# Shigangli/Ok-Topk

Hardware: NVIDIA H100
Metric: train_samples_per_sec_vgg16_oktopk_density0.001 (higher is better)
Workload: dtype fp32

## Files before the change

oktopk_b200/csrc/bindings.cpp:

```cpp
#include <pybind11/pybind11.h>
#include <pybind11/stl.h>
#include <cuda.h>
#include <cuda_runtime.h>

#include <unistd.h>

#include <algorithm>
#include <cstring>
#include <stdexcept>
#include <string>
#include <tuple>
#include <vector>

#include "oktopk.cuh"

namespace py = pybind11;
using namespace okt;

static void ck(cudaError_t e, const char* what) {
    if (e != cudaSuccess) throw std::runtime_error(std::string(what) + ": " + cudaGetErrorString(e));
}
template <class T> static T* P_(uint64_t p) { return reinterpret_cast<T*>(p); }
static cudaStream_t S_(uint64_t s) { return reinterpret_cast<cudaStream_t>(s); }

static py::tuple symm_alloc(size_t nbytes) {
    void* p = nullptr;
    ck(cudaMalloc(&p, nbytes), "cudaMalloc(symm)");
    ck(cudaMemset(p, 0, nbytes), "cudaMemset(symm)");
    cudaIpcMemHandle_t h;
    ck(cudaIpcGetMemHandle(&h, p), "cudaIpcGetMemHandle");
    return py::make_tuple((uint64_t)p, py::bytes(reinterpret_cast<const char*>(&h), sizeof(h)));
}
static uint64_t symm_open(const std::string& handle) {
    if (handle.size() != sizeof(cudaIpcMemHandle_t)) throw std::runtime_error("bad IPC handle size");
    cudaIpcMemHandle_t h;
    std::memcpy(&h, handle.data(), sizeof(h));
    void* p = nullptr;
    ck(cudaIpcOpenMemHandle(&p, h, cudaIpcMemLazyEnablePeerAccess), "cudaIpcOpenMemHandle");
    return (uint64_t)p;
}
static void symm_close(uint64_t p) { ck(cudaIpcCloseMemHandle(P_<void>(p)), "cudaIpcCloseMemHandle"); }
static void symm_free(uint64_t p) { ck(cudaFree(P_<void>(p)), "cudaFree(symm)"); }
static uint64_t dev_alloc_zero(size_t nbytes) {
    void* p = nullptr;
    ck(cudaMalloc(&p, nbytes), "cudaMalloc");
    ck(cudaMemset(p, 0, nbytes), "cudaMemset");
    return (uint64_t)p;
}
static void dev_free(uint64_t p) {
    if (p) ck(cudaFree(P_<void>(p)), "cudaFree");
}
static void memset_async(uint64_t p, int value, size_t nbytes, uint64_t stream) {
    ck(cudaMemsetAsync(P_<void>(p), value, nbytes, S_(stream)), "cudaMemsetAsync");
}
static int can_access_peer(int dev, int peer) {
    int ok = 0;
    ck(cudaDeviceCanAccessPeer(&ok, dev, peer), "cudaDeviceCanAccessPeer");
    return ok;
}


namespace drv {
template <class F> static F sym(const char* name) {
    void* fn = nullptr;
    cudaDriverEntryPointQueryResult q;
    cudaError_t e = cudaGetDriverEntryPoint(name, &fn, cudaEnableDefault, &q);
    if (e != cudaSuccess || fn == nullptr || q != cudaDriverEntryPointSuccess)
        throw std::runtime_error(std::string("driver entry point not available: ") + name);
    return reinterpret_cast<F>(fn);
}
static void ckd(CUresult r, const char* what) {
    if (r != CUDA_SUCCESS) throw std::runtime_error(std::string(what) + ": CUresult " + std::to_string((int)r));
}
}

static CUmemAllocationProp vmm_prop(int dev) {
    CUmemAllocationProp prop;
    std::memset(&prop, 0, sizeof(prop));
    prop.type = CU_MEM_ALLOCATION_TYPE_PINNED;
    prop.location.type = CU_MEM_LOCATION_TYPE_DEVICE;
    prop.location.id = dev;
    prop.requestedHandleTypes = CU_MEM_HANDLE_TYPE_POSIX_FILE_DESCRIPTOR;
    return prop;
}

static py::dict vmm_probe(int dev, int ndev) {
    py::dict d;
    d["vmm"] = 0; d["posix_fd"] = 0; d["multicast"] = 0; d["granularity"] = 0; d["mc_granularity"] = 0;
    try {
        auto getattr_ = drv::sym<CUresult (*)(int*, CUdevice_attribute, CUdevice)>("cuDeviceGetAttribute");
        int v = 0;
        if (getattr_(&v, CU_DEVICE_ATTRIBUTE_VIRTUAL_MEMORY_MANAGEMENT_SUPPORTED, dev) == CUDA_SUCCESS) d["vmm"] = v;
        if (getattr_(&v, CU_DEVICE_ATTRIBUTE_HANDLE_TYPE_POSIX_FILE_DESCRIPTOR_SUPPORTED, dev) == CUDA_SUCCESS) d["posix_fd"] = v;
        if (getattr_(&v, CU_DEVICE_ATTRIBUTE_MULTICAST_SUPPORTED, dev) == CUDA_SUCCESS) d["multicast"] = v;
        auto gran = drv::sym<CUresult (*)(size_t*, const CUmemAllocationProp*, CUmemAllocationGranularity_flags)>("cuMemGetAllocationGranularity");
        CUmemAllocationProp prop = vmm_prop(dev);
        size_t g = 0;
        if (gran(&g, &prop, CU_MEM_ALLOC_GRANULARITY_RECOMMENDED) == CUDA_SUCCESS) d["granularity"] = g;
        if (d["multicast"].cast<int>() && ndev > 1) {
            auto mgran = drv::sym<CUresult (*)(size_t*, const CUmulticastObjectProp*, CUmulticastGranularity_flags)>("cuMulticastGetGranularity");
            CUmulticastObjectProp mp;
            std::memset(&mp, 0, sizeof(mp));
            mp.numDevices = ndev; mp.size = 1 << 21; mp.handleTypes = CU_MEM_HANDLE_TYPE_POSIX_FILE_DESCRIPTOR;
            size_t mg = 0;
            if (mgran(&mg, &mp, CU_MULTICAST_GRANULARITY_RECOMMENDED) == CUDA_SUCCESS) d["mc_granularity"] = mg;
        }
    } catch (const std::exception& e) {
        d["error"] = std::string(e.what());
    }
    return d;
}

static py::tuple vmm_create(size_t nbytes, int dev) {
    auto create = drv::sym<CUresult (*)(CUmemGenericAllocationHandle*, size_t, const CUmemAllocationProp*, unsigned long long)>("cuMemCreate");
    auto exp = drv::sym<CUresult (*)(void*, CUmemGenericAllocationHandle, CUmemAllocationHandleType, unsigned long long)>("cuMemExportToShareableHandle");
    CUmemAllocationProp prop = vmm_prop(dev);
    CUmemGenericAllocationHandle h = 0;
    drv::ckd(create(&h, nbytes, &prop, 0), "cuMemCreate");
    int fd = -1;
    drv::ckd(exp(&fd, h, CU_MEM_HANDLE_TYPE_POSIX_FILE_DESCRIPTOR, 0), "cuMemExportToShareableHandle");
    return py::make_tuple((uint64_t)h, fd);
}
static uint64_t vmm_import(int fd) {
    auto imp = drv::sym<CUresult (*)(CUmemGenericAllocationHandle*, void*, CUmemAllocationHandleType)>("cuMemImportFromShareableHandle");
    CUmemGenericAllocationHandle h = 0;
    drv::ckd(imp(&h, reinterpret_cast<void*>(static_cast<uintptr_t>(fd)), CU_MEM_HANDLE_TYPE_POSIX_FILE_DESCRIPTOR), "cuMemImportFromShareableHandle");
    return (uint64_t)h;
}
static uint64_t vmm_map(uint64_t handle, size_t nbytes, int dev, size_t align) {
    auto reserve = drv::sym<CUresult (*)(CUdeviceptr*, size_t, size_t, CUdeviceptr, unsigned long long)>("cuMemAddressReserve");
    auto map = drv::sym<CUresult (*)(CUdeviceptr, size_t, size_t, CUmemGenericAllocationHandle, unsigned long long)>("cuMemMap");
    auto access = drv::sym<CUresult (*)(CUdeviceptr, size_t, const CUmemAccessDesc*, size_t)>("cuMemSetAccess");
    CUdeviceptr va = 0;
    drv::ckd(reserve(&va, nbytes, align, 0, 0), "cuMemAddressReserve");
    drv::ckd(map(va, nbytes, 0, (CUmemGenericAllocationHandle)handle, 0), "cuMemMap");
    CUmemAccessDesc ad;
    std::memset(&ad, 0, sizeof(ad));
    ad.location.type = CU_MEM_LOCATION_TYPE_DEVICE;
    ad.location.id = dev;
    ad.flags = CU_MEM_ACCESS_FLAGS_PROT_READWRITE;
    drv::ckd(access(va, nbytes, &ad, 1), "cuMemSetAccess");
    return (uint64_t)va;
}
static void vmm_unmap(uint64_t va, size_t nbytes) {
    auto unmap = drv::sym<CUresult (*)(CUdeviceptr, size_t)>("cuMemUnmap");
    auto afree = drv::sym<CUresult (*)(CUdeviceptr, size_t)>("cuMemAddressFree");
    unmap((CUdeviceptr)va, nbytes);
    afree((CUdeviceptr)va, nbytes);
}
static void vmm_release(uint64_t handle) {
    auto rel = drv::sym<CUresult (*)(CUmemGenericAllocationHandle)>("cuMemRelease");
    rel((CUmemGenericAllocationHandle)handle);
}
static py::tuple mc_create(size_t nbytes, int ndev) {
    auto create = drv::sym<CUresult (*)(CUmemGenericAllocationHandle*, const CUmulticastObjectProp*)>("cuMulticastCreate");
    auto exp = drv::sym<CUresult (*)(void*, CUmemGenericAllocationHandle, CUmemAllocationHandleType, unsigned long long)>("cuMemExportToShareableHandle");
    CUmulticastObjectProp mp;
    std::memset(&mp, 0, sizeof(mp));
    mp.numDevices = ndev; mp.size = nbytes; mp.handleTypes = CU_MEM_HANDLE_TYPE_POSIX_FILE_DESCRIPTOR;
    CUmemGenericAllocationHandle h = 0;
    drv::ckd(create(&h, &mp), "cuMulticastCreate");
    int fd = -1;
    drv::ckd(exp(&fd, h, CU_MEM_HANDLE_TYPE_POSIX_FILE_DESCRIPTOR, 0), "cuMemExportToShareableHandle(mc)");
    return py::make_tuple((uint64_t)h, fd);
}
static void mc_add_device(uint64_t mc, int dev) {
    auto add = drv::sym<CUresult (*)(CUmemGenericAllocationHandle, CUdevice)>("cuMulticastAddDevice");
    drv::ckd(add((CUmemGenericAllocationHandle)mc, dev), "cuMulticastAddDevice");
}
static void mc_bind(uint64_t mc, uint64_t mem, size_t nbytes) {
    auto bind = drv::sym<CUresult (*)(CUmemGenericAllocationHandle, size_t, CUmemGenericAllocationHandle, size_t, size_t, unsigned long long)>("cuMulticastBindMem");
    drv::ckd(bind((CUmemGenericAllocationHandle)mc, 0, (CUmemGenericAllocationHandle)mem, 0, nbytes, 0), "cuMulticastBindMem");
}

static size_t state_bytes() { return sizeof(OktState); }

static py::dict layout_info(int P, int n, int cap, int gcap) {
    SymmLayout L = make_layout(P, n, cap, gcap);
    py::dict d;
    d["total"] = L.total; d["rs_mbox"] = L.rs_mbox; d["rs_thr"] = L.rs_thr; d["ag_mbox"] = L.ag_mbox;
    d["cut_mbox"] = L.cut_mbox; d["cut_data"] = L.cut_data; d["send_idx"] = L.send_idx; d["send_val"] = L.send_val;
    d["gat_idx"] = L.gat_idx; d["gat_val"] = L.gat_val; d["cap"] = L.cap; d["gcap"] = L.gcap; d["scap"] = L.scap;
    d["done_mbox"] = L.done_mbox; d["tree_mbox"] = L.tree_mbox;
    d["chunk"] = kChunk; d["maxp"] = OKT_MAXP; d["threads"] = kThreads;
    return d;
}

static py::dict read_state(uint64_t st, int P, uint64_t stream) {
    static thread_local std::vector<char> host(offsetof(OktState, hist));
    ck(cudaMemcpyAsync(host.data(), P_<void>(st), host.size(), cudaMemcpyDeviceToHost, S_(stream)), "read_state");
    ck(cudaStreamSynchronize(S_(stream)), "read_state sync");
    const OktState* s = reinterpret_cast<const OktState*>(host.data());
    py::dict d;
    d["local_thr"] = s->local_thr; d["local_thr_used"] = s->local_thr_used; d["global_thr"] = s->global_thr;
    d["epoch"] = s->epoch;
    std::vector<int> e(s->edges, s->edges + P + 1);
    d["edges"] = e;
    d["local_count"] = s->stat_local_count; d["global_count"] = s->stat_global_count;
    d["recv_total"] = s->stat_recv_total; d["gather_total"] = s->stat_gather_total;
    d["overflow_send"] = s->stat_overflow_send; d["overflow_gather"] = s->stat_overflow_gather;
    d["redo"] = s->stat_redo; d["dense_fallback"] = s->stat_dense_fallback; d["pack_thr"] = s->pack_thr;
    d["cum_overflow_send"] = s->cum_overflow_send; d["cum_overflow_gather"] = s->cum_overflow_gather;
    d["cum_redo"] = s->cum_redo;
    d["fault"] = s->fault;
    auto us = [&](int a, int b) { return s->t_phase[b] >= s->t_phase[a] ? (double)(s->t_phase[b] - s->t_phase[a]) * 1e-3 : 0.0; };
    py::dict ph;
    ph["local"] = us(5, 0); ph["pack"] = us(0, 1); ph["wait_rs"] = us(1, 6); ph["reduce"] = us(6, 2); ph["gselect"] = us(2, 3);
    ph["wait_ag"] = us(3, 7); ph["final"] = us(7, 4); ph["total"] = us(5, 4);
    d["phase_us"] = ph;
    return d;
}

static py::list read_trace(uint64_t st, uint64_t stream) {
    std::vector<TraceRec> host(kTraceLen);
    ck(cudaMemcpyAsync(host.data(), reinterpret_cast<char*>(P_<OktState>(st)) + offsetof(OktState, trace),
                       sizeof(TraceRec) * kTraceLen, cudaMemcpyDeviceToHost, S_(stream)), "read_trace");
    ck(cudaStreamSynchronize(S_(stream)), "read_trace sync");
    py::list out;
    for (const TraceRec& t : host) {
        if (t.epoch == 0) continue;
        py::dict d;
        d["epoch"] = t.epoch; d["local_count"] = t.local_count; d["global_count"] = t.global_count;
        d["recv_total"] = t.recv_total; d["gather_total"] = t.gather_total; d["overflow_send"] = t.overflow_send;
        d["overflow_gather"] = t.overflow_gather; d["redo"] = t.redo; d["local_thr"] = t.local_thr;
        d["global_thr"] = t.global_thr; d["us_local"] = t.us_local; d["us_pack"] = t.us_pack;
        d["us_wait_rs"] = t.us_wait_rs; d["us_reduce"] = t.us_reduce; d["us_gselect"] = t.us_gselect;
        d["us_wait_ag"] = t.us_wait_ag; d["us_final"] = t.us_final; d["t_begin"] = t.t_begin;
        out.append(d);
    }
    return out;
}

static py::tuple host_flag_alloc() {
    int* h = nullptr;
    ck(cudaHostAlloc(reinterpret_cast<void**>(&h), sizeof(int) * 16, cudaHostAllocMapped), "cudaHostAlloc(flag)");
    for (int i = 0; i < 16; ++i) h[i] = 0;
    void* d = nullptr;
    ck(cudaHostGetDevicePointer(&d, h, 0), "cudaHostGetDevicePointer");
    return py::make_tuple((uint64_t)h, (uint64_t)d);
}
static void host_flag_free(uint64_t h) { if (h) cudaFreeHost(P_<void>(h)); }
static int host_flag_read(uint64_t h) { return h ? *reinterpret_cast<volatile int*>(h) : 0; }
static void host_flag_clear(uint64_t h) { if (h) *reinterpret_cast<volatile int*>(h) = 0; }

static void write_state(uint64_t st, float local_thr, float global_thr, const std::vector<int>& edges, uint64_t stream) {
    std::vector<char> host(offsetof(OktState, hist));
    ck(cudaMemcpyAsync(host.data(), P_<void>(st), host.size(), cudaMemcpyDeviceToHost, S_(stream)), "write_state rd");
    ck(cudaStreamSynchronize(S_(stream)), "write_state sync");
    OktState* s = reinterpret_cast<OktState*>(host.data());
    s->local_thr = local_thr;
    s->global_thr = global_thr;
    if (!edges.empty()) {
        if (edges.size() > OKT_MAXP + 1) throw std::runtime_error("too many region edges");
        for (size_t i = 0; i < edges.size(); ++i) s->edges[i] = edges[i];
    }
    ck(cudaMemcpyAsync(P_<void>(st), host.data(), host.size(), cudaMemcpyHostToDevice, S_(stream)), "write_state wr");
    ck(cudaStreamSynchronize(S_(stream)), "write_state sync2");
}

static void fill_peers(char** dst, const std::vector<uint64_t>& peers) {
    if (peers.size() > OKT_MAXP) throw std::runtime_error("world larger than OKT_MAXP");
    for (int i = 0; i < OKT_MAXP; ++i) dst[i] = nullptr;
    for (size_t i = 0; i < peers.size(); ++i) dst[i] = P_<char>(peers[i]);
}

static void oktopk_run(uint64_t g, uint64_t res, uint64_t st, const std::vector<uint64_t>& peers, int n, int rank,
                       int k, int cap, int gcap, py::dict o, int grid, uint64_t stream) {
    OktParams p;
    std::memset(&p, 0, sizeof(p));
    p.g = P_<float>(g); p.res = P_<float>(res); p.st = P_<OktState>(st);
    if (!o.contains("cand") || !o.contains("ccap")) throw std::runtime_error("oktopk_run: candidate scratch missing");
    p.cand = P_<int>(o["cand"].cast<uint64_t>()); p.ccap = o["ccap"].cast<int>();
    p.cand_mode = o.contains("cand_mode") ? o["cand_mode"].cast<int>() : 1;
    fill_peers(p.peers, peers);
    p.P = (int)peers.size(); p.rank = rank; p.n = n; p.k = k;
    p.L = make_layout(p.P, n, cap, gcap);
    auto geti = [&](const char* key, int dflt) { return o.contains(key) ? o[key].cast<int>() : dflt; };
    auto getf = [&](const char* key, double dflt) { return o.contains(key) ? o[key].cast<double>() : dflt; };
    for (int i = 0; i < OKT_MAXP; ++i) p.peer_g[i] = nullptr;
    if (o.contains("peer_g")) {
        auto pg = o["peer_g"].cast<std::vector<uint64_t>>();
        for (size_t i = 0; i < pg.size() && i < OKT_MAXP; ++i) p.peer_g[i] = P_<float>(pg[i]);
    }
    p.max_redo = geti("max_redo", 12);
    p.redo_factor = (float)getf("redo_factor", 1.5);
    p.dense_nnz_limit = geti("dense_nnz_limit", 0);
    p.host_fault = o.contains("host_fault") ? P_<int>(o["host_fault"].cast<uint64_t>()) : nullptr;
    p.trace = geti("trace", 0);
    p.exact_local = geti("exact_local", 0);
    p.repartition = geti("repartition", 0);
    p.uniform_regions = geti("uniform_regions", 0);
    p.residual_mode = geti("residual_mode", RES_OKTOPK);
    p.global_mode = geti("global_mode", GLB_THRESHOLD);
    p.deterministic = geti("deterministic", 0);
    p.pull_tma = geti("pull_tma", 1);
    p.phase_begin = geti("phase_begin", 0);
    p.phase_end = geti("phase_end", PH_END);
    p.guard_loops = geti("guard_loops", 0);
    if (p.guard_loops > kGuardFineMax) p.guard_loops = kGuardFineMax;
    p.cap_limit = geti("cap_limit", 0);
    p.cap_rungs = geti("cap_rungs", 40);
    p.cap_factor = (float)getf("cap_factor", 1.19);
    p.guard_limit = geti("guard_limit", 0);
    p.guard_factor = (float)getf("guard_factor", 1.03);
    p.l_low_cnt = getf("l_low_cnt", 0.0); p.l_high_cnt = getf("l_high_cnt", 1e30);
    p.l_factor = (float)getf("l_factor", 1.012);
    p.g_low_cnt = getf("g_low_cnt", 0.0); p.g_high_cnt = getf("g_high_cnt", 1e30);
    p.g_inc = (float)getf("g_inc", 1.008); p.g_dec = (float)getf("g_dec", 1.008);
    p.prefilter = (float)getf("prefilter", 0.8);
    p.timeout_ns = (unsigned long long)(getf("timeout_s", 0.0) * 1e9);
    if (o.contains("srcs")) {
        auto t = o["srcs"].cast<std::tuple<std::vector<uint64_t>, std::vector<long long>, std::vector<long long>>>();
        const auto& ptr = std::get<0>(t);
        const auto& off = std::get<1>(t);
        const auto& len = std::get<2>(t);
        if (off.size() != ptr.size() || len.size() != ptr.size()) throw std::runtime_error("oktopk_run: srcs table size mismatch");
        if (ptr.size() > (size_t)kSrcSegMax) throw std::runtime_error("oktopk_run: more gradient sources than kSrcSegMax");
        long long end = 0;
        for (size_t i = 0; i < ptr.size(); ++i) {
            if (off[i] < end || (off[i] & 3) || len[i] <= 0 || off[i] + len[i] > n || (ptr[i] & 15))
                throw std::runtime_error("oktopk_run: gradient sources must be 16-byte aligned, in bucket order, "
                                         "non-overlapping, at offsets that are multiples of 4 elements");
            p.src[i] = P_<const float>(ptr[i]);
            p.src_off[i] = (int)off[i];
            p.src_len[i] = (int)len[i];
            end = off[i] + len[i];
        }
        p.nsrc = (int)ptr.size();
        p.zero_g = 0;
    } else {
        if (g & 15) throw std::runtime_error("oktopk_run: the bucket must be 16-byte aligned");
        p.src[0] = P_<const float>(g);
        p.src_off[0] = 0;
        p.src_len[0] = n;
        p.nsrc = 1;
        p.zero_g = 1;
    }
    if (geti("split_phases", 0)) {
        for (int ph = p.phase_begin; ph < p.phase_end; ++ph) {
            OktParams q = p;
            q.phase_begin = ph; q.phase_end = ph + 1;
            ck(launch_oktopk(q, grid, S_(stream)), "oktopk phase launch");
        }
    } else {
        ck(launch_oktopk(p, grid, S_(stream)), "oktopk fused launch");
    }
}

static void gather_run(uint64_t g, uint64_t res, uint64_t st, const std::vector<uint64_t>& peers, int n, int rank,
                       int k, int cap, int gcap, py::dict o, int grid, uint64_t stream) {
    GatherParams p;
    std::memset(&p, 0, sizeof(p));
    p.g = P_<float>(g); p.res = P_<float>(res); p.st = P_<OktState>(st);
    fill_peers(p.peers, peers);
    p.P = (int)peers.size(); p.rank = rank; p.n = n; p.k = k;
    p.L = make_layout(p.P, n, cap, gcap);
    p.reselect = o.contains("reselect") ? o["reselect"].cast<int>() : 0;
    p.clip_max_norm = o.contains("clip_max_norm") ? (float)o["clip_max_norm"].cast<double>() : 0.f;
    p.bitmap = o.contains("bitmap") ? P_<unsigned>(o["bitmap"].cast<uint64_t>()) : nullptr;
    p.cand = o.contains("cand") ? P_<int>(o["cand"].cast<uint64_t>()) : nullptr;
    p.ccap = o.contains("ccap") ? o["ccap"].cast<int>() : 0;
    p.host_fault = o.contains("host_fault") ? P_<int>(o["host_fault"].cast<uint64_t>()) : nullptr;
    if (p.reselect && (p.bitmap == nullptr || p.cand == nullptr || p.ccap <= 0))
        throw std::runtime_error("gather_run: TopkA2 needs the bitmap and candidate scratch");
    p.select_mode = o["select_mode"].cast<int>();
    p.exact_now = o.contains("exact_now") ? o["exact_now"].cast<int>() : 0;
    p.gauss_mode = o.contains("gauss_mode") ? o["gauss_mode"].cast<int>() : 0;
    p.gauss_loops = o.contains("gauss_loops") ? o["gauss_loops"].cast<int>() : 20;
    p.gauss_factor = o.contains("gauss_factor") ? (float)o["gauss_factor"].cast<double>() : 1.02f;
    p.density = (float)o["density"].cast<double>();
    p.pull_tma = o.contains("pull_tma") ? o["pull_tma"].cast<int>() : 1;
    p.timeout_ns = o.contains("timeout_s") ? (unsigned long long)(o["timeout_s"].cast<double>() * 1e9) : 0ULL;
    ck(launch_gather_scheme(p, grid, S_(stream)), "gather scheme launch");
}

static void gtopk_run(uint64_t g, uint64_t res, uint64_t st, const std::vector<uint64_t>& peers, int n, int rank,
                      int k, int cap, int gcap, py::dict o, int grid, uint64_t stream) {
    TreeParams p;
    std::memset(&p, 0, sizeof(p));
    p.g = P_<float>(g); p.res = P_<float>(res); p.st = P_<OktState>(st);
    fill_peers(p.peers, peers);
    p.P = (int)peers.size(); p.rank = rank; p.n = n; p.k = k;
    if (p.P & (p.P - 1)) throw std::runtime_error("gTopk needs a power-of-two world size (VGG/allreducer.py:113)");
    p.L = make_layout(p.P, n, cap, gcap);
    p.pull_tma = o.contains("pull_tma") ? o["pull_tma"].cast<int>() : 1;
    p.timeout_ns = o.contains("timeout_s") ? (unsigned long long)(o["timeout_s"].cast<double>() * 1e9) : 0ULL;
    p.clip_max_norm = o.contains("clip_max_norm") ? (float)o["clip_max_norm"].cast<double>() : 0.f;
    p.bitmap = P_<unsigned>(o["bitmap"].cast<uint64_t>());
    p.cand = P_<int>(o["cand"].cast<uint64_t>());
    p.ccap = o["ccap"].cast<int>();
    p.sel_idx = P_<int>(o["sel_idx"].cast<uint64_t>());
    p.sel_val = P_<float>(o["sel_val"].cast<uint64_t>());
    p.selcap = o["selcap"].cast<int>();
    p.host_fault = o.contains("host_fault") ? P_<int>(o["host_fault"].cast<uint64_t>()) : nullptr;
    ck(launch_gtopk(p, grid, S_(stream)), "gtopk launch");
}

static void land_grads(const std::vector<uint64_t>& srcs, const std::vector<long long>& offs, const std::vector<int>& numels,
                       uint64_t bucket, uint64_t stream) {
    const size_t T = srcs.size();
    if (offs.size() != T || numels.size() != T) throw std::runtime_error("land_grads: table size mismatch");
    constexpr int per = 8192;
    for (size_t b = 0; b < T; b += kLandMax) {
        LandParams lp;
        std::memset(&lp, 0, sizeof(lp));
        const int cnt = (int)std::min<size_t>(kLandMax, T - b);
        int blk = 0;
        for (int i = 0; i < cnt; ++i) {
            lp.src[i] = P_<const float>(srcs[b + i]);
            lp.dst_off[i] = offs[b + i];
            lp.numel[i] = numels[b + i];
            lp.blk_begin[i] = blk;
            blk += std::max(1, (numels[b + i] + per - 1) / per);
        }
        lp.blk_begin[cnt] = blk;
        lp.count = cnt;
        ck(launch_land(lp, P_<float>(bucket), S_(stream)), "land_grads");
    }
}

static void dense_run(const std::vector<uint64_t>& bufs, const std::vector<uint64_t>& flags, uint64_t epoch, int n,
                      int rank, int grid, uint64_t stream, uint64_t st, double timeout_s, uint64_t mc,
                      uint64_t host_fault) {
    DenseParams p;
    std::memset(&p, 0, sizeof(p));
    if (bufs.size() > OKT_MAXP || bufs.size() != flags.size()) throw std::runtime_error("bad peer tables");
    for (size_t i = 0; i < bufs.size(); ++i) { p.bufs[i] = P_<float>(bufs[i]); p.flags[i] = P_<uint64_t>(flags[i]); }
    p.epoch = P_<unsigned long long>(epoch);
    p.n = n; p.P = (int)bufs.size(); p.rank = rank; p.scale = 1.0f / (float)p.P;
    p.fault = st ? &P_<OktState>(st)->fault : nullptr;
    p.timeout_ns = (unsigned long long)(timeout_s * 1e9);
    p.mc = P_<float>(mc);
    p.host_fault = P_<int>(host_fault);
    ck(launch_dense_allreduce(p, grid, S_(stream)), "dense allreduce launch");
}

static void kth_abs(uint64_t x, int n, int k, uint64_t st, uint64_t out, int grid, uint64_t stream) {
    ck(launch_kth_abs(P_<float>(x), n, k, P_<OktState>(st), P_<float>(out), grid, S_(stream)), "kth_abs launch");
}

static void fused_sgd(uint64_t p, uint64_t g, uint64_t mom, int n, double lr, double momentum, double dampening,
                      double wd, int nesterov, int first, int zero_grad, double grad_scale, uint64_t stream,
                      uint64_t lr_ptr, uint64_t fault_ptr) {
    ck(launch_fused_sgd(P_<float>(p), P_<float>(g), P_<float>(mom), n, (float)lr, (float)momentum, (float)dampening,
                        (float)wd, nesterov, first, zero_grad, (float)grad_scale, P_<float>(lr_ptr), P_<int>(fault_ptr),
                        S_(stream)),
       "fused_sgd");
}
static void fused_bert_adam(uint64_t p, uint64_t g, uint64_t m, uint64_t v, int n, double lr, double b1, double b2,
                            double eps, double wd, int zero_grad, uint64_t stream, uint64_t lr_ptr, uint64_t fault_ptr) {
    ck(launch_fused_bert_adam(P_<float>(p), P_<float>(g), P_<float>(m), P_<float>(v), n, (float)lr, (float)b1,
                              (float)b2, (float)eps, (float)wd, zero_grad, P_<float>(lr_ptr), P_<int>(fault_ptr),
                              S_(stream)),
       "fused_bert_adam");
}
static void bn_forward(uint64_t x, uint64_t y, uint64_t arg, uint64_t partial, uint64_t gamma, uint64_t beta, uint64_t cbias,
                       uint64_t save_mean, uint64_t save_invstd, uint64_t rmean, uint64_t rvar, uint64_t nbt, double momentum,
                       double eps, int relu, int M, int C, int W, int slot, int max_ctas, uint64_t stream) {
    if (C % 4 != 0) throw std::runtime_error("bn_forward: channel count must be a multiple of 4");
    if (slot < 0) throw std::runtime_error("bn_forward: negative slot");
    ck(launch_bn_forward(P_<const float>(x), P_<float>(y), P_<unsigned char>(arg), P_<float>(partial), P_<const float>(gamma),
                         P_<const float>(beta), P_<const float>(cbias), P_<float>(save_mean), P_<float>(save_invstd),
                         P_<float>(rmean), P_<float>(rvar), P_<long long>(nbt), (float)momentum, (float)eps, relu, M, C, W, slot,
                         max_ctas, S_(stream)), "bn_forward");
}
static void bn_backward(uint64_t x, uint64_t dy, uint64_t arg, uint64_t dx, uint64_t partial, uint64_t gamma, uint64_t beta,
                        uint64_t save_mean, uint64_t save_invstd, uint64_t dgamma, uint64_t dbeta, int relu, int M, int C, int W,
                        int slot, int max_ctas, uint64_t stream) {
    if (slot < 0) throw std::runtime_error("bn_backward: negative slot");
    ck(launch_bn_backward(P_<const float>(x), P_<const float>(dy), P_<const unsigned char>(arg), P_<float>(dx), P_<float>(partial),
                          P_<const float>(gamma), P_<const float>(beta), P_<const float>(save_mean), P_<const float>(save_invstd),
                          P_<float>(dgamma), P_<float>(dbeta), relu, M, C, W, slot, max_ctas, S_(stream)), "bn_backward");
}
static void maxpool2_fwd(uint64_t x, uint64_t y, uint64_t arg, int N, int H, int W, int C, uint64_t stream) {
    if ((C % 4) || (H % 2) || (W % 2)) throw std::runtime_error("maxpool2_fwd: needs C % 4 == 0 and even H, W");
    ck(launch_maxpool2_fwd(P_<const float>(x), P_<float>(y), P_<unsigned char>(arg), N, H, W, C, S_(stream)), "maxpool2_fwd");
}
static void maxpool2_bwd(uint64_t dy, uint64_t arg, uint64_t dx, int N, int H, int W, int C, uint64_t stream) {
    ck(launch_maxpool2_bwd(P_<const float>(dy), P_<const unsigned char>(arg), P_<float>(dx), N, H, W, C, S_(stream)), "maxpool2_bwd");
}
static void momentum_correct(uint64_t g, uint64_t buf, int n, double momentum, uint64_t stream) {
    ck(launch_momentum_correct(P_<float>(g), P_<float>(buf), n, (float)momentum, S_(stream)), "momentum_correct");
}
static void clip_by_norm(uint64_t x, int n, uint64_t scratch, double max_norm, uint64_t stream) {
    ck(launch_l2norm_sq(P_<float>(x), n, P_<float>(scratch), S_(stream)), "l2norm");
    ck(launch_scale(P_<float>(x), n, P_<float>(scratch), (float)max_norm, S_(stream)), "clip scale");
}

PYBIND11_MODULE(_C, m) {
    m.doc() = "oktopk_b200 native extension (sm_90a kernels + symmetric peer memory)";
    m.def("symm_alloc", &symm_alloc);
    m.def("symm_open", &symm_open);
    m.def("symm_close", &symm_close);
    m.def("symm_free", &symm_free);
    m.def("dev_alloc_zero", &dev_alloc_zero);
    m.def("dev_free", &dev_free);
    m.def("memset_async", &memset_async);
    m.def("can_access_peer", &can_access_peer);
    m.def("state_bytes", &state_bytes);
    m.def("layout_info", &layout_info);
    m.def("read_state", &read_state);
    m.def("write_state", &write_state);
    m.def("max_coop_grid", &okt_max_coop_grid);
    m.def("oktopk_run", &oktopk_run);
    m.def("gather_run", &gather_run);
    m.def("dense_run", &dense_run, py::arg("bufs"), py::arg("flags"), py::arg("epoch"), py::arg("n"), py::arg("rank"),
          py::arg("grid"), py::arg("stream"), py::arg("st") = 0, py::arg("timeout_s") = 0.0, py::arg("mc") = 0,
          py::arg("host_fault") = 0);
    m.def("gtopk_run", &gtopk_run);
    m.def("land_grads", &land_grads);
    m.def("read_trace", &read_trace);
    m.def("host_flag_alloc", &host_flag_alloc);
    m.def("host_flag_free", &host_flag_free);
    m.def("host_flag_read", &host_flag_read);
    m.def("host_flag_clear", &host_flag_clear);
    m.def("fault_ptr", [](uint64_t st) { return (uint64_t)&P_<OktState>(st)->fault; });
    m.def("gather_max_coop_grid", &gather_max_coop_grid);
    m.def("gtopk_max_coop_grid", &gtopk_max_coop_grid);
    m.def("vmm_probe", &vmm_probe);
    m.def("vmm_create", &vmm_create);
    m.def("vmm_import", &vmm_import);
    m.def("vmm_map", &vmm_map);
    m.def("vmm_unmap", &vmm_unmap);
    m.def("vmm_release", &vmm_release);
    m.def("mc_create", &mc_create);
    m.def("mc_add_device", &mc_add_device);
    m.def("mc_bind", &mc_bind);
    m.def("close_fd", [](int fd) { if (fd >= 0) ::close(fd); });
    m.def("clear_fault", [](uint64_t st, uint64_t stream) {
        ck(cudaMemsetAsync(&P_<OktState>(st)->fault, 0, sizeof(int), S_(stream)), "clear_fault");
    });
    m.def("kth_abs", &kth_abs);
    m.def("fused_sgd", &fused_sgd, py::arg("p"), py::arg("g"), py::arg("mom"), py::arg("n"), py::arg("lr"),
          py::arg("momentum"), py::arg("dampening"), py::arg("wd"), py::arg("nesterov"), py::arg("first"),
          py::arg("zero_grad"), py::arg("grad_scale"), py::arg("stream"), py::arg("lr_ptr") = 0, py::arg("fault_ptr") = 0);
    m.def("fused_bert_adam", &fused_bert_adam, py::arg("p"), py::arg("g"), py::arg("m"), py::arg("v"), py::arg("n"),
          py::arg("lr"), py::arg("b1"), py::arg("b2"), py::arg("eps"), py::arg("wd"), py::arg("zero_grad"),
          py::arg("stream"), py::arg("lr_ptr") = 0, py::arg("fault_ptr") = 0);
    m.def("momentum_correct", &momentum_correct);
    m.def("maxpool2_fwd", &maxpool2_fwd);
    m.def("maxpool2_bwd", &maxpool2_bwd);
    m.def("bn_forward", &bn_forward);
    m.def("bn_backward", &bn_backward);
    m.def("bn_tile_rows", &bn_tile_rows);
    m.def("clip_by_norm", &clip_by_norm);
    m.attr("MAXP") = OKT_MAXP;
    m.attr("TRACE_LEN") = kTraceLen;
    m.attr("LAND_MAX") = kLandMax;
    m.attr("SRC_SEG_MAX") = kSrcSegMax;
    m.attr("CHUNK") = kChunk;
}
```

oktopk_b200/csrc/bnrelu.cu:

```cuda
#include "common.cuh"
#include "oktopk.cuh"

namespace okt {

constexpr int kBnThreads = 256;
constexpr int kBnMaxBlocks = 512;
constexpr int kBnHold = 8;
constexpr int kBnSyncSlots = 1024;

__device__ unsigned int g_bn_sync[kBnSyncSlots][2];

struct BnGeom {
    int M, C, cv;
    int tpr, rpi;
    int rows_per_block, nblk;
    int hold;
    int W;
};

__host__ __device__ inline BnGeom bn_geom(int M, int C) {
    BnGeom g;
    g.M = M; g.C = C; g.cv = C >> 2;
    g.tpr = g.cv < kBnThreads ? g.cv : kBnThreads;
    g.rpi = kBnThreads / g.tpr;
    if (g.rpi < 1) g.rpi = 1;
    long long want = ((long long)M * C + 8191) / 8192;
    if (want < 1) want = 1;
    if (want > kBnMaxBlocks) want = kBnMaxBlocks;
    int rpb = (int)((M + want - 1) / want);
    rpb = (rpb + g.rpi - 1) / g.rpi * g.rpi;
    if (rpb < g.rpi) rpb = g.rpi;
    g.rows_per_block = rpb;
    g.nblk = (M + rpb - 1) / rpb;
    g.hold = g.cv <= kBnThreads && rpb / g.rpi <= kBnHold;
    g.W = 0;
    return g;
}

__device__ __forceinline__ float4 f4_fma(const float4& x, const float4& a, const float4& b) {
    return make_float4(fmaf(x.x, a.x, b.x), fmaf(x.y, a.y, b.y), fmaf(x.z, a.z, b.z), fmaf(x.w, a.w, b.w));
}

__device__ __forceinline__ void pool_step(float4& m, uchar4& a, const float4& v, unsigned char k) {
    if (v.x > m.x || v.x != v.x) { m.x = v.x; a.x = k; }
    if (v.y > m.y || v.y != v.y) { m.y = v.y; a.y = k; }
    if (v.z > m.z || v.z != v.z) { m.z = v.z; a.z = k; }
    if (v.w > m.w || v.w != v.w) { m.w = v.w; a.w = k; }
}

__device__ __forceinline__ void bn_combine_partials(const float* __restrict__ partial, int nblk, int C, float* s_tot,
                                                    float4* s_scr) {
    const int cols = (2 * C) >> 2;
    const float4* p4 = reinterpret_cast<const float4*>(partial);
    for (int c0 = 0; c0 < cols; c0 += kBnThreads) {
        const int w = min(kBnThreads, cols - c0);
        const int groups = kBnThreads / w;
        const int tx = threadIdx.x % w, ty = threadIdx.x / w;
        float4 acc = make_float4(0.f, 0.f, 0.f, 0.f);
        if (ty < groups)
            for (int b0 = ty; b0 < nblk; b0 += 8 * groups) {
                float4 v[8];
#pragma unroll
                for (int u = 0; u < 8; ++u)
                    if (b0 + u * groups < nblk) v[u] = __ldcg(p4 + (size_t)(b0 + u * groups) * cols + c0 + tx);
#pragma unroll
                for (int u = 0; u < 8; ++u)
                    if (b0 + u * groups < nblk) { acc.x += v[u].x; acc.y += v[u].y; acc.z += v[u].z; acc.w += v[u].w; }
            }
        s_scr[threadIdx.x] = acc;
        __syncthreads();
        if (ty == 0) {
            for (int j = 1; j < groups; ++j) {
                const float4 v = s_scr[j * w + tx];
                acc.x += v.x; acc.y += v.y; acc.z += v.z; acc.w += v.w;
            }
            reinterpret_cast<float4*>(s_tot)[c0 + tx] = acc;
        }
        __syncthreads();
    }
}

__device__ __forceinline__ void bn_tile_partial(float4 s, float4 q, int tx, int ty, int col, const BnGeom& g, float4* s_red,
                                                float* __restrict__ partial, int tile) {
    if (ty < g.rpi) { s_red[ty * g.tpr + tx] = s; s_red[(g.rpi + ty) * g.tpr + tx] = q; }
    __syncthreads();
    if (ty == 0 && col < g.cv) {
        for (int j = 1; j < g.rpi; ++j) {
            const float4 a = s_red[j * g.tpr + tx], b = s_red[(g.rpi + j) * g.tpr + tx];
            s.x += a.x; s.y += a.y; s.z += a.z; s.w += a.w;
            q.x += b.x; q.y += b.y; q.z += b.z; q.w += b.w;
        }
        float4* p4 = reinterpret_cast<float4*>(partial + (size_t)tile * 2 * g.C);
        p4[col] = s;
        p4[g.cv + col] = q;
    }
    __syncthreads();
}

__device__ __forceinline__ bool bn_arrive(unsigned int* sync, unsigned int& gen) {
    __shared__ unsigned int s_gen;
    __shared__ int s_last;
    __syncthreads();
    if (threadIdx.x == 0) {
        s_gen = ld_acquire_gpu_u32(sync + 1);
        const unsigned int old = atom_add_acq_rel_gpu_u32(sync, 1u);
        s_last = old == gridDim.x - 1u;
        if (s_last) st_relaxed_gpu_u32(sync, 0u);
    }
    __syncthreads();
    gen = s_gen;
    return s_last != 0;
}

__device__ __forceinline__ void bn_release(unsigned int* sync, bool last, unsigned int gen) {
    __syncthreads();
    if (threadIdx.x == 0) {
        if (last) {
            st_release_gpu_u32(sync + 1, gen + 1u);
        } else {
            while (ld_acquire_gpu_u32(sync + 1) == gen) { }
        }
    }
    __syncthreads();
}

struct BnFwdArgs {
    const float* x;
    float* y;
    unsigned char* arg;
    float* partial;
    const float* gamma; const float* beta; const float* cbias;
    float* save_mean; float* save_invstd; float* rmean; float* rvar; long long* nbt;
    float momentum, eps;
    int relu;
    unsigned int* sync;
    BnGeom g;
};

template <bool kPool>
__global__ void __launch_bounds__(kBnThreads) bn_fwd_kernel(const BnFwdArgs p) {
    extern __shared__ float4 s_dyn[];
    __shared__ float4 s_red[2 * kBnThreads];
    const BnGeom& g = p.g;
    const int tx = threadIdx.x % g.tpr, ty = threadIdx.x / g.tpr;
    const float4* x4 = reinterpret_cast<const float4*>(p.x);
    const size_t st1 = (size_t)g.rpi * g.cv;
    float4 h[kBnHold];

    for (int t = blockIdx.x; t < g.nblk; t += gridDim.x) {
        const bool held = g.hold && t == (int)blockIdx.x;
        const int row0 = t * g.rows_per_block, row1 = min(g.M, row0 + g.rows_per_block);
        for (int c0 = 0; c0 < g.cv; c0 += g.tpr) {
            const int col = c0 + tx;
            float4 s = make_float4(0.f, 0.f, 0.f, 0.f), q = s;
            if (ty < g.rpi && col < g.cv) {
                auto acc = [&](const float4& v) {
                    s.x += v.x; s.y += v.y; s.z += v.z; s.w += v.w;
                    q.x = fmaf(v.x, v.x, q.x); q.y = fmaf(v.y, v.y, q.y); q.z = fmaf(v.z, v.z, q.z); q.w = fmaf(v.w, v.w, q.w);
                };
                int r = row0 + ty;
                if (held) {
#pragma unroll
                    for (int k = 0; k < kBnHold; ++k)
                        h[k] = r + k * g.rpi < row1 ? __ldg(x4 + (size_t)(r + k * g.rpi) * g.cv + col) : make_float4(0.f, 0.f, 0.f, 0.f);
#pragma unroll
                    for (int k = 0; k < kBnHold; ++k)
                        if (r + k * g.rpi < row1) acc(h[k]);
                } else {
                    for (; r + 3 * g.rpi < row1; r += 4 * g.rpi) {
                        const float4* q0 = x4 + (size_t)r * g.cv + col;
                        const float4 v0 = __ldg(q0), v1 = __ldg(q0 + st1), v2 = __ldg(q0 + 2 * st1), v3 = __ldg(q0 + 3 * st1);
                        acc(v0); acc(v1); acc(v2); acc(v3);
                    }
                    for (; r < row1; r += g.rpi) acc(__ldg(x4 + (size_t)r * g.cv + col));
                }
            }
            bn_tile_partial(s, q, tx, ty, col, g, s_red, p.partial, t);
        }
    }

    float* s_ab = reinterpret_cast<float*>(s_dyn);
    unsigned int gen;
    const bool last = bn_arrive(p.sync, gen);
    if (last) {
        float* s_tot = s_ab;
        bn_combine_partials(p.partial, g.nblk, g.C, s_tot, s_red);
        for (int c = threadIdx.x; c < g.C; c += kBnThreads) {
            const double s = (double)s_tot[c], q = (double)s_tot[g.C + c];
            const double mean = s / (double)g.M;
            double var = q / (double)g.M - mean * mean;
            if (var < 0.0) var = 0.0;
            const float invstd = (float)(1.0 / sqrt(var + (double)p.eps));
            p.save_mean[c] = (float)mean;
            p.save_invstd[c] = invstd;
            if (p.rmean != nullptr) {
                const float mb = (float)mean + (p.cbias != nullptr ? __ldg(p.cbias + c) : 0.f);
                const double unb = g.M > 1 ? var * (double)g.M / (double)(g.M - 1) : var;
                p.rmean[c] = fmaf(p.momentum, mb, __fmul_rn(1.f - p.momentum, p.rmean[c]));
                p.rvar[c] = fmaf(p.momentum, (float)unb, __fmul_rn(1.f - p.momentum, p.rvar[c]));
            }
        }
        if (threadIdx.x == 0 && p.nbt != nullptr) *p.nbt += 1;
    }
    bn_release(p.sync, last, gen);
    for (int c = threadIdx.x; c < g.C; c += kBnThreads) {
        const float a = __fmul_rn(__ldg(p.gamma + c), __ldcg(p.save_invstd + c));
        s_ab[c] = a;
        s_ab[g.C + c] = __fsub_rn(__ldg(p.beta + c), __fmul_rn(__ldcg(p.save_mean + c), a));
    }
    __syncthreads();

    const float4* ab4 = s_dyn;
    auto yval = [&](const float4& xin, int col) {
        float4 v = f4_fma(xin, ab4[col], ab4[g.cv + col]);
        if (p.relu) { v.x = fmaxf(v.x, 0.f); v.y = fmaxf(v.y, 0.f); v.z = fmaxf(v.z, 0.f); v.w = fmaxf(v.w, 0.f); }
        return v;
    };
    float4* y4 = reinterpret_cast<float4*>(p.y);
    for (int t = blockIdx.x; t < g.nblk; t += gridDim.x) {
        const bool held = g.hold && t == (int)blockIdx.x;
        const int row0 = t * g.rows_per_block, row1 = min(g.M, row0 + g.rows_per_block);
        if (!kPool) {
            for (int c0 = 0; c0 < g.cv; c0 += g.tpr) {
                const int col = c0 + tx;
                if (ty >= g.rpi || col >= g.cv) continue;
                int r = row0 + ty;
                if (held) {
#pragma unroll
                    for (int k = 0; k < kBnHold; ++k)
                        if (r + k * g.rpi < row1) y4[(size_t)(r + k * g.rpi) * g.cv + col] = yval(h[k], col);
                    continue;
                }
                for (; r + 3 * g.rpi < row1; r += 4 * g.rpi) {
                    const size_t o = (size_t)r * g.cv + col;
                    const float4 v0 = __ldg(x4 + o), v1 = __ldg(x4 + o + st1), v2 = __ldg(x4 + o + 2 * st1), v3 = __ldg(x4 + o + 3 * st1);
                    y4[o] = yval(v0, col); y4[o + st1] = yval(v1, col); y4[o + 2 * st1] = yval(v2, col); y4[o + 3 * st1] = yval(v3, col);
                }
                for (; r < row1; r += g.rpi) { const size_t o = (size_t)r * g.cv + col; y4[o] = yval(__ldg(x4 + o), col); }
            }
        } else {
            float4* sy = s_dyn + g.C / 2;
            if (held) {
                if (ty < g.rpi) {
#pragma unroll
                    for (int k = 0; k < kBnHold; ++k)
                        if (row0 + ty + k * g.rpi < row1) sy[(ty + k * g.rpi) * g.cv + tx] = yval(h[k], tx);
                }
                __syncthreads();
            }
            auto at = [&](int lr, int c) { return held ? sy[lr * g.cv + c] : yval(__ldg(x4 + (size_t)(row0 + lr) * g.cv + c), c); };
            const int W = g.W, Wo = W >> 1, npool = (row1 - row0) / 4 * g.cv;
            uchar4* a4 = reinterpret_cast<uchar4*>(p.arg);
            for (int i = threadIdx.x; i < npool; i += kBnThreads) {
                const int c = i % g.cv, pp = i / g.cv;
                const int lr = (pp / Wo) * 2 * W + (pp % Wo) * 2;
                const float4 v1 = at(lr + 1, c), v2 = at(lr + W, c), v3 = at(lr + W + 1, c);
                float4 m = at(lr, c);
                uchar4 a = make_uchar4(0, 0, 0, 0);
                pool_step(m, a, v1, 1);
                pool_step(m, a, v2, 2);
                pool_step(m, a, v3, 3);
                const size_t o = (size_t)(row0 / 4 + pp) * g.cv + c;
                y4[o] = m;
                a4[o] = a;
            }
        }
    }
}

struct BnBwdArgs {
    const float* x;
    const float* dy;
    const unsigned char* arg;
    float* dx;
    float* partial;
    const float* gamma; const float* beta; const float* save_mean; const float* save_invstd;
    float* dgamma; float* dbeta;
    int relu;
    unsigned int* sync;
    BnGeom g;
};

template <bool kPool>
__global__ void __launch_bounds__(kBnThreads) bn_bwd_kernel(const BnBwdArgs p) {
    extern __shared__ float4 s_dyn[];
    __shared__ float4 s_red[2 * kBnThreads];
    const BnGeom& g = p.g;
    const int tx = threadIdx.x % g.tpr, ty = threadIdx.x / g.tpr;
    const float4* x4 = reinterpret_cast<const float4*>(p.x);
    const float4* d4 = reinterpret_cast<const float4*>(p.dy);
    const uchar4* a4 = reinterpret_cast<const uchar4*>(p.arg);
    const size_t st1 = (size_t)g.rpi * g.cv;
    auto grad = [&](int row0, int r, int col) -> float4 {
        if (!kPool) return __ldg(d4 + (size_t)r * g.cv + col);
        const int lr = r - row0, hl = lr / g.W, w = lr - hl * g.W;
        const size_t o = (size_t)(row0 / 4 + (hl >> 1) * (g.W >> 1) + (w >> 1)) * g.cv + col;
        const int k = (hl & 1) * 2 + (w & 1);
        const float4 d = __ldg(d4 + o);
        const uchar4 a = __ldg(a4 + o);
        return make_float4(a.x == k ? d.x : 0.f, a.y == k ? d.y : 0.f, a.z == k ? d.z : 0.f, a.w == k ? d.w : 0.f);
    };
    struct Col { float4 mean, istd, a, b; };
    auto column = [&](int col) {
        Col k;
        k.mean = __ldg(reinterpret_cast<const float4*>(p.save_mean) + col);
        k.istd = __ldg(reinterpret_cast<const float4*>(p.save_invstd) + col);
        const float4 gm = __ldg(reinterpret_cast<const float4*>(p.gamma) + col);
        const float4 bt = __ldg(reinterpret_cast<const float4*>(p.beta) + col);
        k.a = make_float4(__fmul_rn(gm.x, k.istd.x), __fmul_rn(gm.y, k.istd.y), __fmul_rn(gm.z, k.istd.z), __fmul_rn(gm.w, k.istd.w));
        k.b = make_float4(__fsub_rn(bt.x, __fmul_rn(k.mean.x, k.a.x)), __fsub_rn(bt.y, __fmul_rn(k.mean.y, k.a.y)),
                          __fsub_rn(bt.z, __fmul_rn(k.mean.z, k.a.z)), __fsub_rn(bt.w, __fmul_rn(k.mean.w, k.a.w)));
        return k;
    };
    auto mask = [&](const Col& k, const float4& v, float4& d) {
        if (p.relu) {
            if (!(fmaf(v.x, k.a.x, k.b.x) > 0.f)) d.x = 0.f;
            if (!(fmaf(v.y, k.a.y, k.b.y) > 0.f)) d.y = 0.f;
            if (!(fmaf(v.z, k.a.z, k.b.z) > 0.f)) d.z = 0.f;
            if (!(fmaf(v.w, k.a.w, k.b.w) > 0.f)) d.w = 0.f;
        }
    };
    auto xhat = [&](const Col& k, const float4& v) {
        return make_float4((v.x - k.mean.x) * k.istd.x, (v.y - k.mean.y) * k.istd.y, (v.z - k.mean.z) * k.istd.z,
                           (v.w - k.mean.w) * k.istd.w);
    };
    float4 hx[kBnHold], hd[kBnHold];

    for (int t = blockIdx.x; t < g.nblk; t += gridDim.x) {
        const bool held = g.hold && t == (int)blockIdx.x;
        const int row0 = t * g.rows_per_block, row1 = min(g.M, row0 + g.rows_per_block);
        for (int c0 = 0; c0 < g.cv; c0 += g.tpr) {
            const int col = c0 + tx;
            float4 sb = make_float4(0.f, 0.f, 0.f, 0.f), sg = sb;
            if (ty < g.rpi && col < g.cv) {
                const Col k = column(col);
                auto acc = [&](const float4& v, float4 d) {
                    const float4 xh = xhat(k, v);
                    mask(k, v, d);
                    sb.x += d.x; sb.y += d.y; sb.z += d.z; sb.w += d.w;
                    sg.x = fmaf(d.x, xh.x, sg.x); sg.y = fmaf(d.y, xh.y, sg.y); sg.z = fmaf(d.z, xh.z, sg.z); sg.w = fmaf(d.w, xh.w, sg.w);
                };
                int r = row0 + ty;
                if (held) {
#pragma unroll
                    for (int j = 0; j < kBnHold; ++j) {
                        const int rr = r + j * g.rpi;
                        hx[j] = rr < row1 ? __ldg(x4 + (size_t)rr * g.cv + col) : make_float4(0.f, 0.f, 0.f, 0.f);
                        hd[j] = rr < row1 ? grad(row0, rr, col) : make_float4(0.f, 0.f, 0.f, 0.f);
                    }
#pragma unroll
                    for (int j = 0; j < kBnHold; ++j)
                        if (r + j * g.rpi < row1) acc(hx[j], hd[j]);
                } else {
                    for (; r + 3 * g.rpi < row1; r += 4 * g.rpi) {
                        const size_t o = (size_t)r * g.cv + col;
                        const float4 v0 = __ldg(x4 + o), v1 = __ldg(x4 + o + st1), v2 = __ldg(x4 + o + 2 * st1), v3 = __ldg(x4 + o + 3 * st1);
                        const float4 e0 = grad(row0, r, col), e1 = grad(row0, r + g.rpi, col), e2 = grad(row0, r + 2 * g.rpi, col),
                                     e3 = grad(row0, r + 3 * g.rpi, col);
                        acc(v0, e0); acc(v1, e1); acc(v2, e2); acc(v3, e3);
                    }
                    for (; r < row1; r += g.rpi) acc(__ldg(x4 + (size_t)r * g.cv + col), grad(row0, r, col));
                }
            }
            bn_tile_partial(sb, sg, tx, ty, col, g, s_red, p.partial, t);
        }
    }

    unsigned int gen;
    const bool last = bn_arrive(p.sync, gen);
    if (last) {
        float* s_tot = reinterpret_cast<float*>(s_dyn);
        bn_combine_partials(p.partial, g.nblk, g.C, s_tot, s_red);
        for (int c = threadIdx.x; c < g.C; c += kBnThreads) { p.dbeta[c] = s_tot[c]; p.dgamma[c] = s_tot[g.C + c]; }
    }
    bn_release(p.sync, last, gen);

    for (int t = blockIdx.x; t < g.nblk; t += gridDim.x) {
        const bool held = g.hold && t == (int)blockIdx.x;
        const int row0 = t * g.rows_per_block, row1 = min(g.M, row0 + g.rows_per_block);
        for (int c0 = 0; c0 < g.cv; c0 += g.tpr) {
            const int col = c0 + tx;
            if (ty >= g.rpi || col >= g.cv) continue;
            const Col k = column(col);
            const float4 db = __ldcg(reinterpret_cast<const float4*>(p.dbeta) + col);
            const float4 dg = __ldcg(reinterpret_cast<const float4*>(p.dgamma) + col);
            const double M = (double)g.M;
            const float4 mb = make_float4((float)(db.x / M), (float)(db.y / M), (float)(db.z / M), (float)(db.w / M));
            const float4 mg = make_float4((float)(dg.x / M), (float)(dg.y / M), (float)(dg.z / M), (float)(dg.w / M));
            float4* o4 = reinterpret_cast<float4*>(p.dx);
            auto out = [&](size_t off, const float4& v, float4 d) {
                const float4 xh = xhat(k, v);
                mask(k, v, d);
                o4[off] = make_float4(k.a.x * (d.x - mb.x - xh.x * mg.x), k.a.y * (d.y - mb.y - xh.y * mg.y),
                                      k.a.z * (d.z - mb.z - xh.z * mg.z), k.a.w * (d.w - mb.w - xh.w * mg.w));
            };
            int r = row0 + ty;
            if (held) {
#pragma unroll
                for (int j = 0; j < kBnHold; ++j)
                    if (r + j * g.rpi < row1) out((size_t)(r + j * g.rpi) * g.cv + col, hx[j], hd[j]);
                continue;
            }
            for (; r + 3 * g.rpi < row1; r += 4 * g.rpi) {
                const size_t o = (size_t)r * g.cv + col;
                const float4 v0 = __ldg(x4 + o), v1 = __ldg(x4 + o + st1), v2 = __ldg(x4 + o + 2 * st1), v3 = __ldg(x4 + o + 3 * st1);
                const float4 e0 = grad(row0, r, col), e1 = grad(row0, r + g.rpi, col), e2 = grad(row0, r + 2 * g.rpi, col),
                             e3 = grad(row0, r + 3 * g.rpi, col);
                out(o, v0, e0); out(o + st1, v1, e1); out(o + 2 * st1, v2, e2); out(o + 3 * st1, v3, e3);
            }
            for (; r < row1; r += g.rpi) out((size_t)r * g.cv + col, __ldg(x4 + (size_t)r * g.cv + col), grad(row0, r, col));
        }
    }
}

int bn_tile_rows(int M, int C) { return bn_geom(M, C).rows_per_block; }

static unsigned int* bn_sync_slot(int slot) {
    static unsigned int* base[64] = {nullptr};
    int dev = 0;
    cudaGetDevice(&dev);
    if (dev < 0 || dev >= 64) return nullptr;
    if (base[dev] == nullptr) {
        void* a = nullptr;
        if (cudaGetSymbolAddress(&a, g_bn_sync) != cudaSuccess) return nullptr;
        base[dev] = static_cast<unsigned int*>(a);
    }
    return base[dev] + 2 * (size_t)(slot % kBnSyncSlots);
}

template <typename Args>
static cudaError_t bn_launch(void (*kernel)(const Args), Args p, size_t smem, int max_ctas, cudaStream_t stream) {
    int dev = 0, sms = 0, per = 0;
    cudaGetDevice(&dev);
    cudaError_t e = cudaDeviceGetAttribute(&sms, cudaDevAttrMultiProcessorCount, dev);
    if (e == cudaSuccess && smem > 32 * 1024)
        e = cudaFuncSetAttribute(kernel, cudaFuncAttributeMaxDynamicSharedMemorySize, (int)smem);
    if (e == cudaSuccess) e = cudaOccupancyMaxActiveBlocksPerMultiprocessor(&per, kernel, kBnThreads, smem);
    if (e != cudaSuccess) return e;
    if (per < 1) return cudaErrorInvalidConfiguration;
    int grid = p.g.nblk < per * sms ? p.g.nblk : per * sms;
    if (max_ctas > 0 && grid > max_ctas) grid = max_ctas;
    void* args[] = {(void*)&p};
    e = cudaLaunchCooperativeKernel((void*)kernel, dim3(grid), dim3(kBnThreads), args, smem, stream);
    (void)cudaGetLastError();
    return e;
}

static cudaError_t bn_prepare(BnGeom& g, unsigned int*& sync, int M, int C, int W, int slot) {
    g = bn_geom(M, C);
    g.W = W;
    if (W > 0 && (W % 2 != 0 || g.rows_per_block % (2 * W) != 0 || M % (2 * W) != 0)) return cudaErrorInvalidValue;
    sync = bn_sync_slot(slot);
    return sync == nullptr ? cudaErrorInvalidDevice : cudaSuccess;
}

cudaError_t launch_bn_forward(const float* x, float* y, unsigned char* arg, float* partial, const float* gamma, const float* beta,
                              const float* cbias, float* save_mean, float* save_invstd, float* rmean, float* rvar, long long* nbt,
                              float momentum, float eps, int relu, int M, int C, int W, int slot, int max_ctas,
                              cudaStream_t stream) {
    BnFwdArgs p{x, y, arg, partial, gamma, beta, cbias, save_mean, save_invstd, rmean, rvar, nbt, momentum, eps, relu, nullptr, {}};
    cudaError_t e = bn_prepare(p.g, p.sync, M, C, W, slot);
    if (e != cudaSuccess) return e;
    size_t smem = sizeof(float) * 2 * C;
    if (W > 0 && p.g.hold) smem += sizeof(float4) * p.g.rows_per_block * p.g.cv;
    return W > 0 ? bn_launch(bn_fwd_kernel<true>, p, smem, max_ctas, stream) : bn_launch(bn_fwd_kernel<false>, p, smem, max_ctas, stream);
}

cudaError_t launch_bn_backward(const float* x, const float* dy, const unsigned char* arg, float* dx, float* partial,
                               const float* gamma, const float* beta, const float* save_mean, const float* save_invstd,
                               float* dgamma, float* dbeta, int relu, int M, int C, int W, int slot, int max_ctas,
                               cudaStream_t stream) {
    BnBwdArgs p{x, dy, arg, dx, partial, gamma, beta, save_mean, save_invstd, dgamma, dbeta, relu, nullptr, {}};
    cudaError_t e = bn_prepare(p.g, p.sync, M, C, W, slot);
    if (e != cudaSuccess) return e;
    const size_t smem = sizeof(float) * 2 * C;
    return W > 0 ? bn_launch(bn_bwd_kernel<true>, p, smem, max_ctas, stream) : bn_launch(bn_bwd_kernel<false>, p, smem, max_ctas, stream);
}

}

namespace okt {

constexpr int kPoolThreads = 256;

__global__ void __launch_bounds__(kPoolThreads) maxpool2_fwd_kernel(const float* __restrict__ x, float* __restrict__ y,
                                                                     unsigned char* __restrict__ arg, int N, int H, int W,
                                                                     int C) {
    const int cv = C >> 2, Ho = H >> 1, Wo = W >> 1;
    const long long total = (long long)N * Ho * Wo * cv;
    const float4* x4 = reinterpret_cast<const float4*>(x);
    float4* y4 = reinterpret_cast<float4*>(y);
    uchar4* a4 = reinterpret_cast<uchar4*>(arg);
    for (long long t = (long long)blockIdx.x * kPoolThreads + threadIdx.x; t < total; t += (long long)gridDim.x * kPoolThreads) {
        const int c = (int)(t % cv);
        long long p = t / cv;
        const int wo = (int)(p % Wo); p /= Wo;
        const int ho = (int)(p % Ho);
        const int n = (int)(p / Ho);
        const size_t base = (((size_t)n * H + 2 * ho) * W + 2 * wo) * cv + c;
        const float4 v0 = __ldg(x4 + base), v1 = __ldg(x4 + base + cv);
        const float4 v2 = __ldg(x4 + base + (size_t)W * cv), v3 = __ldg(x4 + base + (size_t)W * cv + cv);
        float4 m = v0;
        uchar4 a = make_uchar4(0, 0, 0, 0);
        pool_step(m, a, v1, 1);
        pool_step(m, a, v2, 2);
        pool_step(m, a, v3, 3);
        y4[t] = m;
        a4[t] = a;
    }
}

__global__ void __launch_bounds__(kPoolThreads) maxpool2_bwd_kernel(const float* __restrict__ dy,
                                                                     const unsigned char* __restrict__ arg,
                                                                     float* __restrict__ dx, int N, int H, int W, int C) {
    const int cv = C >> 2, Ho = H >> 1, Wo = W >> 1;
    const long long total = (long long)N * Ho * Wo * cv;
    const float4* d4 = reinterpret_cast<const float4*>(dy);
    const uchar4* a4 = reinterpret_cast<const uchar4*>(arg);
    float4* o4 = reinterpret_cast<float4*>(dx);
    for (long long t = (long long)blockIdx.x * kPoolThreads + threadIdx.x; t < total; t += (long long)gridDim.x * kPoolThreads) {
        const int c = (int)(t % cv);
        long long p = t / cv;
        const int wo = (int)(p % Wo); p /= Wo;
        const int ho = (int)(p % Ho);
        const int n = (int)(p / Ho);
        const size_t base = (((size_t)n * H + 2 * ho) * W + 2 * wo) * cv + c;
        const float4 d = __ldg(d4 + t);
        const uchar4 a = a4[t];
        auto pick = [&](int k) {
            return make_float4(a.x == k ? d.x : 0.f, a.y == k ? d.y : 0.f, a.z == k ? d.z : 0.f, a.w == k ? d.w : 0.f);
        };
        o4[base] = pick(0);
        o4[base + cv] = pick(1);
        o4[base + (size_t)W * cv] = pick(2);
        o4[base + (size_t)W * cv + cv] = pick(3);
    }
}

static inline int pool_grid(long long total) {
    long long g = (total + kPoolThreads - 1) / kPoolThreads;
    if (g < 1) g = 1;
    if (g > kStrideGridMax) g = kStrideGridMax;
    return (int)g;
}

cudaError_t launch_maxpool2_fwd(const float* x, float* y, unsigned char* arg, int N, int H, int W, int C, cudaStream_t stream) {
    const long long total = (long long)N * (H / 2) * (W / 2) * (C / 4);
    maxpool2_fwd_kernel<<<pool_grid(total), kPoolThreads, 0, stream>>>(x, y, arg, N, H, W, C);
    return cudaGetLastError();
}
cudaError_t launch_maxpool2_bwd(const float* dy, const unsigned char* arg, float* dx, int N, int H, int W, int C,
                                cudaStream_t stream) {
    const long long total = (long long)N * (H / 2) * (W / 2) * (C / 4);
    maxpool2_bwd_kernel<<<pool_grid(total), kPoolThreads, 0, stream>>>(dy, arg, dx, N, H, W, C);
    return cudaGetLastError();
}

}
```

oktopk_b200/csrc/oktopk.cuh:

```cuda
#pragma once
#include <cuda_runtime.h>
#include <stdint.h>
#include <stddef.h>

#ifndef OKT_MAXP
#define OKT_MAXP 16
#endif

namespace okt {

constexpr int kThreads = 512;
constexpr int kWarps = kThreads / 32;
constexpr int kChunk = 1024;
constexpr int kHistBins = 2048;
constexpr int kMaxWarpsTotal = 16384;
constexpr int kGuardMax = 64;
constexpr int kGuardFineMax = 15;
constexpr int kCtasPerSm = 1;
constexpr int kPackTile = 2;
constexpr int kPackStages = 4;
constexpr int kPackSmemBytes = kPackStages * 2 * kPackTile * kThreads * 16;
constexpr int kScanStages = 2 * kPackStages;
constexpr int kStrideGridMax = 132 * 8;

constexpr int kTraceLen = 256;
struct TraceRec {
    uint32_t epoch;
    int local_count, global_count, recv_total, gather_total, overflow_send, overflow_gather, redo;
    float local_thr, global_thr;
    float us_local, us_pack, us_wait_rs, us_reduce, us_gselect, us_wait_ag, us_final;
    unsigned long long t_begin;
};

struct OktState {
    unsigned long long bar;
    unsigned int tick[4];
    float local_thr;
    float local_thr_used;
    float global_thr;
    uint32_t epoch;
    int edges[OKT_MAXP + 1];
    int send_cursor[OKT_MAXP];
    int gather_cursor;
    int cand_cursor;
    int guard_counts[kGuardMax];
    uint32_t sel_prefix;
    uint32_t sel_krem;
    int cuts[OKT_MAXP];
    int stat_local_count;
    int stat_global_count;
    int stat_recv_total;
    int stat_gather_total;
    int stat_overflow_send;
    int stat_overflow_gather;
    int stat_redo;
    int stat_dense_fallback;
    int stat_mode;
    int fault;
    float pack_thr;
    unsigned long long cum_overflow_send;
    unsigned long long cum_overflow_gather;
    unsigned long long cum_redo;
    unsigned long long snap_overflow_send;
    unsigned long long snap_overflow_gather;
    unsigned long long snap_redo;
    unsigned long long t_phase[8];
    double gs_sum, gs_sumsq;
    double clip_sumsq;
    uint32_t hist[kHistBins];
    int wcounts[kMaxWarpsTotal];
    TraceRec trace[kTraceLen];
};

struct SymmLayout {
    size_t rs_mbox;
    size_t rs_thr;
    size_t ag_mbox;
    size_t cut_mbox;
    size_t cut_data;
    size_t done_mbox;
    size_t tree_mbox;
    size_t send_idx;
    size_t send_val;
    size_t gat_idx;
    size_t gat_val;
    size_t total;
    int cap;
    int scap;
    int gcap;
};

inline size_t align_up(size_t x, size_t a) { return (x + a - 1) / a * a; }

inline SymmLayout make_layout(int P, int n, int cap, int gcap) {
    SymmLayout L;
    size_t o = 0;
    L.rs_mbox = o;  o += sizeof(uint64_t) * 2 * OKT_MAXP;
    L.rs_thr = o;   o += sizeof(float) * 2 * OKT_MAXP;
    L.ag_mbox = o;  o += sizeof(uint64_t) * 2 * OKT_MAXP;
    L.cut_mbox = o; o += sizeof(uint64_t) * 2 * OKT_MAXP;
    L.cut_data = o; o += sizeof(int) * 2 * OKT_MAXP * OKT_MAXP;
    L.done_mbox = o; o += sizeof(uint64_t) * 2 * OKT_MAXP;
    L.tree_mbox = o; o += sizeof(uint64_t) * 2 * OKT_MAXP;
    o = align_up(o, 1024);
    const size_t scap = cap > 0 ? (size_t)P * cap : align_up((size_t)n, 4) + 4 * (size_t)OKT_MAXP + 1024;
    L.send_idx = o; o += sizeof(int) * scap;   o = align_up(o, 1024);
    L.send_val = o; o += sizeof(float) * scap; o = align_up(o, 1024);
    L.gat_idx = o;  o += sizeof(int) * 2 * (size_t)gcap;      o = align_up(o, 1024);
    L.gat_val = o;  o += sizeof(float) * 2 * (size_t)gcap;    o = align_up(o, 1024);
    L.total = o;
    L.cap = cap;
    L.scap = (int)scap;
    L.gcap = gcap;
    return L;
}

enum Phase : int {
    PH_LOCAL = 0,
    PH_PACK = 1,
    PH_PUBLISH_RS = 2,
    PH_REDUCE = 3,
    PH_GSELECT = 4,
    PH_PUBLISH_AG = 5,
    PH_FINAL = 6,
    PH_END = 7
};

enum ResidualMode : int { RES_OKTOPK = 0, RES_LOCAL_GT = 1, RES_LOCAL_GE = 2 };
enum GlobalMode : int { GLB_THRESHOLD = 0, GLB_EXACT_TOPK = 1, GLB_ALL_NONZERO = 2 };

constexpr int kSrcSegMax = 160;

struct OktParams {
    float* g;
    float* res;
    OktState* st;
    int* cand;
    int ccap;
    int cand_mode;
    float prefilter;
    char* peers[OKT_MAXP];
    float* peer_g[OKT_MAXP];
    SymmLayout L;
    int n, P, rank, k;
    int exact_local, repartition, uniform_regions;
    int residual_mode, global_mode;
    int deterministic, pull_tma;
    int phase_begin, phase_end;
    int guard_loops, guard_limit;
    float guard_factor;
    int cap_limit, cap_rungs;
    float cap_factor;
    double l_low_cnt, l_high_cnt;
    float l_factor;
    double g_low_cnt, g_high_cnt;
    float g_inc, g_dec;
    unsigned long long timeout_ns;
    int max_redo;
    float redo_factor;
    int dense_nnz_limit;
    int* host_fault;
    int trace;
    int zero_g;
    int nsrc;
    int src_off[kSrcSegMax];
    int src_len[kSrcSegMax];
    const float* src[kSrcSegMax];
};
static_assert(sizeof(OktParams) <= 4096, "OktParams must fit the 4 KB kernel-parameter limit");

enum GatherSelect : int { GS_THRESHOLD_REUSE = 0, GS_GAUSSIAN = 1, GS_EXACT_TOPK = 2 };

struct GatherParams {
    float* g;
    float* res;
    OktState* st;
    char* peers[OKT_MAXP];
    SymmLayout L;
    int n, P, rank, k;
    int select_mode;
    int exact_now;
    int gauss_mode;
    int gauss_loops;
    float gauss_factor;
    float density;
    int pull_tma;
    unsigned long long timeout_ns;
    int reselect;
    float clip_max_norm;
    unsigned* bitmap;
    int* cand;
    int ccap;
    int* host_fault;
};

struct TreeParams {
    float* g;
    float* res;
    OktState* st;
    char* peers[OKT_MAXP];
    SymmLayout L;
    int n, P, rank, k;
    int pull_tma;
    unsigned long long timeout_ns;
    float clip_max_norm;
    unsigned* bitmap;
    int* cand;
    int ccap;
    int* sel_idx;
    float* sel_val;
    int selcap;
    int* host_fault;
};

struct DenseParams {
    float* bufs[OKT_MAXP];
    uint64_t* flags[OKT_MAXP];
    unsigned long long* epoch;
    int n, P, rank;
    float scale;
    int* fault;
    unsigned long long timeout_ns;
    float* mc;
    int* host_fault;
};

int okt_max_coop_grid(int device);
cudaError_t launch_oktopk(const OktParams& p, int grid, cudaStream_t stream);
cudaError_t launch_gather_scheme(const GatherParams& p, int grid, cudaStream_t stream);
cudaError_t launch_gtopk(const TreeParams& p, int grid, cudaStream_t stream);
int gtopk_max_coop_grid(int device);
int gather_max_coop_grid(int device);
cudaError_t launch_dense_allreduce(const DenseParams& p, int grid, cudaStream_t stream);
cudaError_t launch_kth_abs(const float* x, int n, int k, OktState* st, float* out_thr, int grid, cudaStream_t stream);
cudaError_t launch_fused_sgd(float* p, float* g, float* mom, int n, float lr, float momentum, float dampening,
                             float weight_decay, int nesterov, int first_step, int zero_grad, float grad_scale,
                             const float* lr_ptr, const int* fault, cudaStream_t stream);
cudaError_t launch_fused_bert_adam(float* p, float* g, float* m, float* v, int n, float lr, float b1, float b2,
                                   float eps, float weight_decay, int zero_grad, const float* lr_ptr,
                                   const int* fault, cudaStream_t stream);
constexpr int kLandMax = 96;
struct LandParams {
    const float* src[kLandMax];
    long long dst_off[kLandMax];
    int numel[kLandMax];
    int blk_begin[kLandMax + 1];
    int count;
};
cudaError_t launch_land(const LandParams& lp, float* bucket, cudaStream_t stream);
int bn_tile_rows(int M, int C);
cudaError_t launch_bn_forward(const float* x, float* y, unsigned char* arg, float* partial, const float* gamma, const float* beta,
                              const float* cbias, float* save_mean, float* save_invstd, float* rmean, float* rvar, long long* nbt,
                              float momentum, float eps, int relu, int M, int C, int W, int slot, int max_ctas,
                              cudaStream_t stream);
cudaError_t launch_bn_backward(const float* x, const float* dy, const unsigned char* arg, float* dx, float* partial,
                               const float* gamma, const float* beta, const float* save_mean, const float* save_invstd,
                               float* dgamma, float* dbeta, int relu, int M, int C, int W, int slot, int max_ctas,
                               cudaStream_t stream);
cudaError_t launch_maxpool2_fwd(const float* x, float* y, unsigned char* arg, int N, int H, int W, int C, cudaStream_t stream);
cudaError_t launch_maxpool2_bwd(const float* dy, const unsigned char* arg, float* dx, int N, int H, int W, int C,
                                cudaStream_t stream);
cudaError_t launch_momentum_correct(float* g, float* buf, int n, float momentum, cudaStream_t stream);
cudaError_t launch_l2norm_sq(const float* x, int n, float* out, cudaStream_t stream);
cudaError_t launch_scale(float* x, int n, const float* norm_sq, float max_norm, cudaStream_t stream);

}
```

oktopk_b200/ops/ext.py:

```python
from __future__ import annotations

import importlib
import os
from typing import Optional

_C = None
_ERR: Optional[BaseException] = None

LAUNCH_COUNT = {"total": 0}
_LAUNCHERS = {"oktopk_run": 1, "gather_run": 1, "gtopk_run": 1, "dense_run": 1, "kth_abs": 1, "fused_sgd": 1,
              "fused_bert_adam": 1, "momentum_correct": 1, "clip_by_norm": 2, "land_grads": 1, "bn_forward": 1, "bn_backward": 1,
              "maxpool2_fwd": 1, "maxpool2_bwd": 1}


class _CountingModule:

    def __init__(self, mod):
        self._mod = mod
        for name, per_call in _LAUNCHERS.items():
            setattr(self, name, self._wrap(getattr(mod, name), name, per_call))

    def _wrap(self, fn, name, per_call):
        def call(*a, **kw):
            n = per_call
            if name == "oktopk_run" and isinstance(a[9], dict) and a[9].get("split_phases"):
                n = 7
            if name == "land_grads":
                n = max(1, (len(a[0]) + 95) // 96)
            LAUNCH_COUNT["total"] += n
            LAUNCH_COUNT[name] = LAUNCH_COUNT.get(name, 0) + n
            return fn(*a, **kw)
        return call

    def __getattr__(self, name):
        return getattr(self._mod, name)


def load(build_if_missing: bool = True):
    global _C, _ERR
    if _C is not None:
        return _C
    try:
        from . import build as _b
        if build_if_missing and _b.needs_build() and os.environ.get("OKTOPK_NO_BUILD", "0") != "1":
            _b.build()
        _C = _CountingModule(importlib.import_module("oktopk_b200._C"))
        _ERR = None
    except Exception as e:
        _ERR = e
        _C = None
    return _C


def available() -> bool:
    return load() is not None


def require():
    c = load()
    if c is None:
        raise RuntimeError("oktopk_b200 native extension (_C) is not available: %r" % (_ERR,))
    return c


class DevPtr:

    def __init__(self, ptr: int, numel: int, typestr: str = "<f4"):
        self.ptr, self.numel, self.typestr = int(ptr), int(numel), typestr

    @property
    def __cuda_array_interface__(self):
        return {"shape": (self.numel,), "typestr": self.typestr, "data": (self.ptr, False), "version": 3,
                "strides": None}


def tensor_from_ptr(ptr: int, numel: int, dtype="float32", device=None):
    import torch
    ts = {"float32": "<f4", "int32": "<i4", "uint8": "|u1", "int64": "<i8"}[dtype]
    dev = device if device is not None else torch.device("cuda", torch.cuda.current_device())
    return torch.as_tensor(DevPtr(ptr, numel, ts), device=dev)
```

oktopk_b200/ops/fused_bn.py:

```python
from __future__ import annotations

import itertools
from typing import Optional

import torch
import torch.nn.functional as F

from . import ext

MAX_CTAS = 0

_SLOTS = itertools.count()


def _sync_slot(bn: torch.nn.BatchNorm2d) -> int:
    s = bn.__dict__.get("_okt_bn_slot")
    if s is None:
        s = bn.__dict__["_okt_bn_slot"] = next(_SLOTS)
    return s


def _fast_path_ok(x: torch.Tensor, bn: torch.nn.BatchNorm2d) -> bool:
    return (x.is_cuda and x.dtype == torch.float32 and x.dim() == 4 and bn.training and bn.affine
            and bn.momentum is not None and x.size(1) % 4 == 0
            and x.is_contiguous(memory_format=torch.channels_last) and ext.available()
            and not torch.is_autocast_enabled())


def _is_2x2(pool: torch.nn.MaxPool2d) -> bool:
    ks = pool.kernel_size if isinstance(pool.kernel_size, tuple) else (pool.kernel_size,) * 2
    st = pool.stride if isinstance(pool.stride, tuple) else (pool.stride,) * 2
    pad = pool.padding if isinstance(pool.padding, tuple) else (pool.padding,) * 2
    dil = pool.dilation if isinstance(pool.dilation, tuple) else (pool.dilation,) * 2
    return ks == (2, 2) and st == (2, 2) and pad == (0, 0) and dil == (1, 1) and not pool.return_indices


def _pool_fusable(x: torch.Tensor, pool: torch.nn.MaxPool2d) -> bool:
    N, C, H, W = x.shape
    return (_is_2x2(pool) and H % 2 == 0 and W % 2 == 0
            and ext.require().bn_tile_rows(N * H * W, C) % (2 * W) == 0)


class _BiasBNReLUPool(torch.autograd.Function):
    @staticmethod
    def forward(ctx, x, gamma, beta, cbias, rmean, rvar, nbt, momentum, eps, relu, pool, slot):
        C = ext.require()
        N, Ch, H, W = x.shape
        M = N * H * W
        if pool:
            y = torch.empty((N, Ch, H // 2, W // 2), dtype=x.dtype, device=x.device, memory_format=torch.channels_last)
            arg = torch.empty(y.numel(), dtype=torch.uint8, device=x.device)
        else:
            y = torch.empty_like(x)
            arg = None
        rows = C.bn_tile_rows(M, Ch)
        partial = torch.empty((M + rows - 1) // rows * 2 * Ch, dtype=torch.float32, device=x.device)
        stats = torch.empty(2 * Ch, dtype=torch.float32, device=x.device)
        s = torch.cuda.current_stream().cuda_stream
        C.bn_forward(x.data_ptr(), y.data_ptr(), 0 if arg is None else arg.data_ptr(), partial.data_ptr(), gamma.data_ptr(),
                     beta.data_ptr(), 0 if cbias is None else cbias.data_ptr(), stats.data_ptr(), stats.data_ptr() + 4 * Ch,
                     0 if rmean is None else rmean.data_ptr(), 0 if rvar is None else rvar.data_ptr(),
                     0 if nbt is None else nbt.data_ptr(), float(momentum), float(eps), int(relu), M, Ch,
                     W if pool else 0, slot, MAX_CTAS, s)
        ctx.save_for_backward(x, gamma, beta, stats, arg)
        ctx.relu, ctx.pool, ctx.slot = bool(relu), bool(pool), slot
        return y

    @staticmethod
    def backward(ctx, dy):
        C = ext.require()
        x, gamma, beta, stats, arg = ctx.saved_tensors
        N, Ch, H, W = x.shape
        M = N * H * W
        if not dy.is_contiguous(memory_format=torch.channels_last):
            dy = dy.contiguous(memory_format=torch.channels_last)
        dx = torch.empty_like(x)
        rows = C.bn_tile_rows(M, Ch)
        partial = torch.empty((M + rows - 1) // rows * 2 * Ch, dtype=torch.float32, device=x.device)
        dgb = torch.empty(2 * Ch, dtype=torch.float32, device=x.device)
        s = torch.cuda.current_stream().cuda_stream
        C.bn_backward(x.data_ptr(), dy.data_ptr(), 0 if arg is None else arg.data_ptr(), dx.data_ptr(), partial.data_ptr(),
                      gamma.data_ptr(), beta.data_ptr(), stats.data_ptr(), stats.data_ptr() + 4 * Ch, dgb.data_ptr(),
                      dgb.data_ptr() + 4 * Ch, int(ctx.relu), M, Ch, W if ctx.pool else 0, ctx.slot, MAX_CTAS, s)
        return dx, dgb[:Ch], dgb[Ch:], None, None, None, None, None, None, None, None, None


def bias_bn_relu(x: torch.Tensor, bn: torch.nn.BatchNorm2d, conv_bias: Optional[torch.Tensor] = None,
                 relu: bool = True, pool: Optional[torch.nn.MaxPool2d] = None) -> torch.Tensor:
    if _fast_path_ok(x, bn):
        track = bn.track_running_stats and bn.running_mean is not None
        fuse = pool is not None and _pool_fusable(x, pool)
        y = _BiasBNReLUPool.apply(x, bn.weight, bn.bias, conv_bias, bn.running_mean if track else None,
                                  bn.running_var if track else None, bn.num_batches_tracked if track else None,
                                  bn.momentum, bn.eps, relu, fuse, _sync_slot(bn))
        return y if pool is None or fuse else max_pool_2x2(y, pool)
    if conv_bias is not None:
        x = x + conv_bias.view(1, -1, 1, 1)
    y = bn(x)
    y = F.relu(y) if relu else y
    return y if pool is None else max_pool_2x2(y, pool)


def conv_bn_relu(x: torch.Tensor, conv: torch.nn.Conv2d, bn: torch.nn.BatchNorm2d, relu: bool = True,
                 pool: Optional[torch.nn.MaxPool2d] = None) -> torch.Tensor:
    if _fast_path_ok_pre(x, conv, bn):
        z = F.conv2d(x, conv.weight, None, conv.stride, conv.padding, conv.dilation, conv.groups)
        if _fast_path_ok(z, bn):
            return bias_bn_relu(z, bn, conv.bias, relu, pool)
        if conv.bias is not None:
            z = z + conv.bias.view(1, -1, 1, 1)
        y = bn(z)
    else:
        y = bn(conv(x))
    y = F.relu(y) if relu else y
    return y if pool is None else max_pool_2x2(y, pool)


def _fast_path_ok_pre(x: torch.Tensor, conv: torch.nn.Conv2d, bn: torch.nn.BatchNorm2d) -> bool:
    return (x.is_cuda and x.dtype == torch.float32 and bn.training and bn.affine and bn.momentum is not None
            and conv.out_channels % 4 == 0 and conv.padding_mode == "zeros" and ext.available()
            and x.is_contiguous(memory_format=torch.channels_last) and not torch.is_autocast_enabled()
            and not isinstance(conv.padding, str))


class _MaxPool2x2(torch.autograd.Function):

    @staticmethod
    def forward(ctx, x):
        C = ext.require()
        N, Ch, H, W = x.shape
        y = torch.empty((N, Ch, H // 2, W // 2), dtype=x.dtype, device=x.device, memory_format=torch.channels_last)
        arg = torch.empty(y.numel(), dtype=torch.uint8, device=x.device)
        C.maxpool2_fwd(x.data_ptr(), y.data_ptr(), arg.data_ptr(), N, H, W, Ch, torch.cuda.current_stream().cuda_stream)
        ctx.save_for_backward(arg)
        ctx.shape = (N, Ch, H, W)
        return y

    @staticmethod
    def backward(ctx, dy):
        C = ext.require()
        (arg,) = ctx.saved_tensors
        N, Ch, H, W = ctx.shape
        if not dy.is_contiguous(memory_format=torch.channels_last):
            dy = dy.contiguous(memory_format=torch.channels_last)
        dx = torch.empty((N, Ch, H, W), dtype=dy.dtype, device=dy.device, memory_format=torch.channels_last)
        C.maxpool2_bwd(dy.data_ptr(), arg.data_ptr(), dx.data_ptr(), N, H, W, Ch, torch.cuda.current_stream().cuda_stream)
        return dx


def max_pool_2x2(x: torch.Tensor, pool: torch.nn.MaxPool2d) -> torch.Tensor:
    if (_is_2x2(pool) and x.is_cuda and x.dtype == torch.float32 and x.dim() == 4 and x.size(1) % 4 == 0
            and x.size(2) % 2 == 0 and x.size(3) % 2 == 0 and x.is_contiguous(memory_format=torch.channels_last)
            and ext.available() and torch.is_grad_enabled() and not torch.is_autocast_enabled()):
        return _MaxPool2x2.apply(x)
    return pool(x)


def run_fused_sequential(seq: torch.nn.Sequential, x: torch.Tensor) -> torch.Tensor:
    mods = list(seq.children())
    i = 0
    while i < len(mods):
        m = mods[i]
        if isinstance(m, torch.nn.Conv2d) and i + 1 < len(mods) and isinstance(mods[i + 1], torch.nn.BatchNorm2d):
            relu = i + 2 < len(mods) and isinstance(mods[i + 2], torch.nn.ReLU)
            j = i + (3 if relu else 2)
            pool = mods[j] if j < len(mods) and isinstance(mods[j], torch.nn.MaxPool2d) else None
            x = conv_bn_relu(x, m, mods[i + 1], relu, pool)
            i = j + (1 if pool is not None else 0)
        elif isinstance(m, torch.nn.MaxPool2d):
            x = max_pool_2x2(x, m)
            i += 1
        elif isinstance(m, torch.nn.AvgPool2d) and m.kernel_size in (1, (1, 1)) and m.stride in (1, (1, 1)):
            i += 1
        else:
            x = m(x)
            i += 1
    return x
```

Baseline: 13320.

## Use thread-block clusters with DSMEM reduction for small BatchNorm fused kernels

Adds a cluster-launched variant of the fused BN forward/backward kernels for layers with at most four row tiles. In this variant the per-tile partial sums stay in shared memory and are combined across CTAs through distributed shared memory and cluster barriers. This replaces the global-memory partials plus the atomic grid barrier of the cooperative launch. Per-channel inputs are also prefetched before the reduction. The risks are lower parallelism for those layers, since only up to four CTAs run, and extra shared memory per CTA.

Measured after the change: 13590, median of 6. 1.02x the previous value.

```diff
diff --git a/oktopk_b200/csrc/bindings.cpp b/oktopk_b200/csrc/bindings.cpp
--- a/oktopk_b200/csrc/bindings.cpp
+++ b/oktopk_b200/csrc/bindings.cpp
@@ -454,23 +454,28 @@
                               S_(stream)),
        "fused_bert_adam");
 }
-static void bn_forward(uint64_t x, uint64_t y, uint64_t arg, uint64_t partial, uint64_t gamma, uint64_t beta, uint64_t cbias,
-                       uint64_t save_mean, uint64_t save_invstd, uint64_t rmean, uint64_t rvar, uint64_t nbt, double momentum,
-                       double eps, int relu, int M, int C, int W, int slot, int max_ctas, uint64_t stream) {
+static py::tuple bn_forward(uint64_t x, uint64_t y, uint64_t arg, uint64_t partial, uint64_t gamma, uint64_t beta, uint64_t cbias,
+                            uint64_t save_mean, uint64_t save_invstd, uint64_t rmean, uint64_t rvar, uint64_t nbt, double momentum,
+                            double eps, int relu, int M, int C, int W, int slot, int max_ctas, int cluster_tiles, uint64_t stream) {
     if (C % 4 != 0) throw std::runtime_error("bn_forward: channel count must be a multiple of 4");
     if (slot < 0) throw std::runtime_error("bn_forward: negative slot");
+    BnLaunch l{0, 0};
     ck(launch_bn_forward(P_<const float>(x), P_<float>(y), P_<unsigned char>(arg), P_<float>(partial), P_<const float>(gamma),
                          P_<const float>(beta), P_<const float>(cbias), P_<float>(save_mean), P_<float>(save_invstd),
                          P_<float>(rmean), P_<float>(rvar), P_<long long>(nbt), (float)momentum, (float)eps, relu, M, C, W, slot,
-                         max_ctas, S_(stream)), "bn_forward");
-}
-static void bn_backward(uint64_t x, uint64_t dy, uint64_t arg, uint64_t dx, uint64_t partial, uint64_t gamma, uint64_t beta,
-                        uint64_t save_mean, uint64_t save_invstd, uint64_t dgamma, uint64_t dbeta, int relu, int M, int C, int W,
-                        int slot, int max_ctas, uint64_t stream) {
+                         max_ctas, cluster_tiles, &l, S_(stream)), "bn_forward");
+    return py::make_tuple(l.ctas, l.cluster);
+}
+static py::tuple bn_backward(uint64_t x, uint64_t dy, uint64_t arg, uint64_t dx, uint64_t partial, uint64_t gamma, uint64_t beta,
+                             uint64_t save_mean, uint64_t save_invstd, uint64_t dgamma, uint64_t dbeta, int relu, int M, int C,
+                             int W, int slot, int max_ctas, int cluster_tiles, uint64_t stream) {
     if (slot < 0) throw std::runtime_error("bn_backward: negative slot");
+    BnLaunch l{0, 0};
     ck(launch_bn_backward(P_<const float>(x), P_<const float>(dy), P_<const unsigned char>(arg), P_<float>(dx), P_<float>(partial),
                           P_<const float>(gamma), P_<const float>(beta), P_<const float>(save_mean), P_<const float>(save_invstd),
-                          P_<float>(dgamma), P_<float>(dbeta), relu, M, C, W, slot, max_ctas, S_(stream)), "bn_backward");
+                          P_<float>(dgamma), P_<float>(dbeta), relu, M, C, W, slot, max_ctas, cluster_tiles, &l, S_(stream)),
+       "bn_backward");
+    return py::make_tuple(l.ctas, l.cluster);
 }
 static void maxpool2_fwd(uint64_t x, uint64_t y, uint64_t arg, int N, int H, int W, int C, uint64_t stream) {
     if ((C % 4) || (H % 2) || (W % 2)) throw std::runtime_error("maxpool2_fwd: needs C % 4 == 0 and even H, W");
diff --git a/oktopk_b200/csrc/bnrelu.cu b/oktopk_b200/csrc/bnrelu.cu
--- a/oktopk_b200/csrc/bnrelu.cu
+++ b/oktopk_b200/csrc/bnrelu.cu
@@ -1,3 +1,7 @@
+#include <map>
+#include <mutex>
+#include <tuple>
+
 #include "common.cuh"
 #include "oktopk.cuh"
 
@@ -48,25 +52,41 @@
     if (v.w > m.w || v.w != v.w) { m.w = v.w; a.w = k; }
 }
 
+__device__ __forceinline__ void acc_add(float4& a, const float4& v) { a.x += v.x; a.y += v.y; a.z += v.z; a.w += v.w; }
+__device__ __forceinline__ void acc_add(float& a, float v) { a += v; }
+
+__device__ __forceinline__ int bn_col_groups(int col, int cols) {
+    const int c0 = col - col % kBnThreads;
+    return kBnThreads / min(kBnThreads, cols - c0);
+}
+
+template <class Load>
+__device__ __forceinline__ auto bn_sum_tiles(Load load, int first, int step, int nblk) {
+    using T = decltype(load(first));
+    T acc{};
+    for (int b0 = first; b0 < nblk; b0 += 8 * step) {
+        T v[8];
+#pragma unroll
+        for (int u = 0; u < 8; ++u)
+            if (b0 + u * step < nblk) v[u] = load(b0 + u * step);
+#pragma unroll
+        for (int u = 0; u < 8; ++u)
+            if (b0 + u * step < nblk) acc_add(acc, v[u]);
+    }
+    return acc;
+}
+
 __device__ __forceinline__ void bn_combine_partials(const float* __restrict__ partial, int nblk, int C, float* s_tot,
                                                     float4* s_scr) {
     const int cols = (2 * C) >> 2;
     const float4* p4 = reinterpret_cast<const float4*>(partial);
     for (int c0 = 0; c0 < cols; c0 += kBnThreads) {
         const int w = min(kBnThreads, cols - c0);
-        const int groups = kBnThreads / w;
+        const int groups = bn_col_groups(c0, cols);
         const int tx = threadIdx.x % w, ty = threadIdx.x / w;
         float4 acc = make_float4(0.f, 0.f, 0.f, 0.f);
         if (ty < groups)
-            for (int b0 = ty; b0 < nblk; b0 += 8 * groups) {
-                float4 v[8];
-#pragma unroll
-                for (int u = 0; u < 8; ++u)
-                    if (b0 + u * groups < nblk) v[u] = __ldcg(p4 + (size_t)(b0 + u * groups) * cols + c0 + tx);
-#pragma unroll
-                for (int u = 0; u < 8; ++u)
-                    if (b0 + u * groups < nblk) { acc.x += v[u].x; acc.y += v[u].y; acc.z += v[u].z; acc.w += v[u].w; }
-            }
+            acc = bn_sum_tiles([&](int b) { return __ldcg(p4 + (size_t)b * cols + c0 + tx); }, ty, groups, nblk);
         s_scr[threadIdx.x] = acc;
         __syncthreads();
         if (ty == 0) {
@@ -97,18 +117,21 @@
     __syncthreads();
 }
 
-__device__ __forceinline__ bool bn_arrive(unsigned int* sync, unsigned int& gen) {
-    __shared__ unsigned int s_gen;
+__device__ __forceinline__ unsigned int bn_gen(const unsigned int* sync) {
+    unsigned int v = 0;
+    if (threadIdx.x == 0) asm volatile("ld.relaxed.gpu.global.u32 %0, [%1];" : "=r"(v) : "l"(sync + 1) : "memory");
+    return v;
+}
+
+__device__ __forceinline__ bool bn_arrive(unsigned int* sync) {
     __shared__ int s_last;
     __syncthreads();
     if (threadIdx.x == 0) {
-        s_gen = ld_acquire_gpu_u32(sync + 1);
         const unsigned int old = atom_add_acq_rel_gpu_u32(sync, 1u);
         s_last = old == gridDim.x - 1u;
         if (s_last) st_relaxed_gpu_u32(sync, 0u);
     }
     __syncthreads();
-    gen = s_gen;
     return s_last != 0;
 }
 
@@ -122,6 +145,59 @@
         }
     }
     __syncthreads();
+}
+
+__device__ __forceinline__ void cluster_arrive() { asm volatile("barrier.cluster.arrive.release.aligned;" ::: "memory"); }
+__device__ __forceinline__ void cluster_wait() { asm volatile("barrier.cluster.wait.acquire.aligned;" ::: "memory"); }
+__device__ __forceinline__ void cluster_sync() { cluster_arrive(); cluster_wait(); }
+
+__device__ __forceinline__ uint32_t dsmem_addr(const void* p, int rank) {
+    uint32_t a;
+    asm volatile("mapa.shared::cluster.u32 %0, %1, %2;" : "=r"(a) : "r"(smem_u32(p)), "r"(rank));
+    return a;
+}
+__device__ __forceinline__ float ld_dsmem_f32(const float* p, int rank) {
+    float v;
+    asm volatile("ld.shared::cluster.f32 %0, [%1];" : "=f"(v) : "r"(dsmem_addr(p, rank)));
+    return v;
+}
+
+struct BnClusterSmem { int per, own, part, end; };
+
+__host__ __device__ inline BnClusterSmem bn_cluster_smem(const BnGeom& g, int base, int ctas) {
+    BnClusterSmem s;
+    s.per = (g.cv + ctas - 1) / ctas;
+    s.own = base;
+    s.part = s.own + 8 * s.per;
+    s.end = s.part + (g.nblk + ctas - 1) / ctas * 2 * g.C;
+    return s;
+}
+
+template <class Fn>
+__device__ __forceinline__ void bn_cluster_combine(const BnGeom& g, const float* s_part, int q0, int per, Fn fn) {
+    const int ctas = gridDim.x, cols = g.cv * 2, c0 = 4 * q0;
+    for (int i0 = 0; i0 < 8 * per; i0 += kBnThreads) {
+        const int i = i0 + threadIdx.x, c = c0 + (i >> 1), h = i & 1;
+        const bool mine = i < 8 * per && c < g.C;
+        float tot = 0.f;
+        if (mine) {
+            const int groups = bn_col_groups(h * g.cv + (c >> 2), cols);
+            const float* col = s_part + h * g.C + c;
+            auto load = [&](int b) { return ld_dsmem_f32(col + (size_t)(b / ctas) * 2 * g.C, b % ctas); };
+            tot = bn_sum_tiles(load, 0, groups, g.nblk);
+            for (int j = 1; j < groups; ++j) tot += bn_sum_tiles(load, j, groups, g.nblk);
+        }
+        const float other = __shfl_xor_sync(0xffffffffu, tot, 1);
+        if (mine && h == 0) fn(c, tot, other);
+    }
+}
+
+__device__ __forceinline__ void bn_cluster_gather(const BnGeom& g, const float* s_own, int per, float* s_out) {
+    for (int c = threadIdx.x; c < g.C; c += kBnThreads) {
+        const int q = c >> 2, owner = q / per, off = (q - owner * per) * 4 + (c & 3);
+        s_out[c] = ld_dsmem_f32(s_own + off, owner);
+        s_out[g.C + c] = ld_dsmem_f32(s_own + 4 * per + off, owner);
+    }
 }
 
 struct BnFwdArgs {
@@ -137,15 +213,67 @@
     BnGeom g;
 };
 
-template <bool kPool>
+struct BnChanIn { float rm, rv, cb, gm, bt; };
+
+__device__ __forceinline__ BnChanIn bn_chan_in(const BnFwdArgs& p, int c) {
+    BnChanIn in;
+    in.rm = p.rmean != nullptr ? p.rmean[c] : 0.f;
+    in.rv = p.rmean != nullptr ? p.rvar[c] : 0.f;
+    in.cb = p.cbias != nullptr ? __ldg(p.cbias + c) : 0.f;
+    in.gm = __ldg(p.gamma + c);
+    in.bt = __ldg(p.beta + c);
+    return in;
+}
+
+__device__ __forceinline__ void bn_channel_stats(const BnFwdArgs& p, int c, const BnChanIn& in, float s_sum, float s_sq,
+                                                 float& mean_f, float& invstd) {
+    const BnGeom& g = p.g;
+    const float rm = in.rm, rv = in.rv, cb = in.cb;
+    const double s = (double)s_sum, q = (double)s_sq;
+    const double mean = s / (double)g.M;
+    double var = q / (double)g.M - mean * mean;
+    if (var < 0.0) var = 0.0;
+    invstd = (float)(1.0 / sqrt(var + (double)p.eps));
+    mean_f = (float)mean;
+    p.save_mean[c] = mean_f;
+    p.save_invstd[c] = invstd;
+    if (p.rmean != nullptr) {
+        const float mb = mean_f + cb;
+        const double unb = g.M > 1 ? var * (double)g.M / (double)(g.M - 1) : var;
+        p.rmean[c] = fmaf(p.momentum, mb, __fmul_rn(1.f - p.momentum, rm));
+        p.rvar[c] = fmaf(p.momentum, (float)unb, __fmul_rn(1.f - p.momentum, rv));
+    }
+}
+
+__device__ __forceinline__ void bn_affine(float gamma, float beta, float mean, float invstd, float& a, float& b) {
+    a = __fmul_rn(gamma, invstd);
+    b = __fsub_rn(beta, __fmul_rn(mean, a));
+}
+
+template <bool kPool, bool kCluster>
 __global__ void __launch_bounds__(kBnThreads) bn_fwd_kernel(const BnFwdArgs p) {
     extern __shared__ float4 s_dyn[];
     __shared__ float4 s_red[2 * kBnThreads];
     const BnGeom& g = p.g;
+    const BnClusterSmem cs = bn_cluster_smem(g, 2 * g.C + (kPool && g.hold ? 4 * g.rows_per_block * g.cv : 0), gridDim.x);
+    float* s_part = reinterpret_cast<float*>(s_dyn) + cs.part;
     const int tx = threadIdx.x % g.tpr, ty = threadIdx.x / g.tpr;
     const float4* x4 = reinterpret_cast<const float4*>(p.x);
     const size_t st1 = (size_t)g.rpi * g.cv;
     float4 h[kBnHold];
+
+    constexpr int kBnPre = 2;
+    const unsigned int gen = kCluster ? 0u : bn_gen(p.sync);
+    const long long nbt0 = threadIdx.x == 0 && p.nbt != nullptr ? *p.nbt : 0;
+    BnChanIn pre[kBnPre];
+    const int c_own = kCluster ? 4 * (int)blockIdx.x * cs.per + (int)(threadIdx.x >> 1) : 0;
+    if (kCluster) {
+        if ((threadIdx.x & 1) == 0 && c_own < min(g.C, 4 * ((int)blockIdx.x + 1) * cs.per)) pre[0] = bn_chan_in(p, c_own);
+    } else {
+#pragma unroll
+        for (int k = 0; k < kBnPre; ++k)
+            if (threadIdx.x + k * kBnThreads < g.C) pre[k] = bn_chan_in(p, threadIdx.x + k * kBnThreads);
+    }
 
     for (int t = blockIdx.x; t < g.nblk; t += gridDim.x) {
         const bool held = g.hold && t == (int)blockIdx.x;
@@ -175,38 +303,46 @@
                     for (; r < row1; r += g.rpi) acc(__ldg(x4 + (size_t)r * g.cv + col));
                 }
             }
-            bn_tile_partial(s, q, tx, ty, col, g, s_red, p.partial, t);
+            if (kCluster) bn_tile_partial(s, q, tx, ty, col, g, s_red, s_part, t / gridDim.x);
+            else bn_tile_partial(s, q, tx, ty, col, g, s_red, p.partial, t);
         }
     }
 
     float* s_ab = reinterpret_cast<float*>(s_dyn);
-    unsigned int gen;
-    const bool last = bn_arrive(p.sync, gen);
-    if (last) {
-        float* s_tot = s_ab;
-        bn_combine_partials(p.partial, g.nblk, g.C, s_tot, s_red);
-        for (int c = threadIdx.x; c < g.C; c += kBnThreads) {
-            const double s = (double)s_tot[c], q = (double)s_tot[g.C + c];
-            const double mean = s / (double)g.M;
-            double var = q / (double)g.M - mean * mean;
-            if (var < 0.0) var = 0.0;
-            const float invstd = (float)(1.0 / sqrt(var + (double)p.eps));
-            p.save_mean[c] = (float)mean;
-            p.save_invstd[c] = invstd;
-            if (p.rmean != nullptr) {
-                const float mb = (float)mean + (p.cbias != nullptr ? __ldg(p.cbias + c) : 0.f);
-                const double unb = g.M > 1 ? var * (double)g.M / (double)(g.M - 1) : var;
-                p.rmean[c] = fmaf(p.momentum, mb, __fmul_rn(1.f - p.momentum, p.rmean[c]));
-                p.rvar[c] = fmaf(p.momentum, (float)unb, __fmul_rn(1.f - p.momentum, p.rvar[c]));
-            }
-        }
-        if (threadIdx.x == 0 && p.nbt != nullptr) *p.nbt += 1;
-    }
-    bn_release(p.sync, last, gen);
-    for (int c = threadIdx.x; c < g.C; c += kBnThreads) {
-        const float a = __fmul_rn(__ldg(p.gamma + c), __ldcg(p.save_invstd + c));
-        s_ab[c] = a;
-        s_ab[g.C + c] = __fsub_rn(__ldg(p.beta + c), __fmul_rn(__ldcg(p.save_mean + c), a));
+    if (kCluster) {
+        float* s_own = reinterpret_cast<float*>(s_dyn) + cs.own;
+        const int q0 = blockIdx.x * cs.per;
+        cluster_sync();
+        bn_cluster_combine(g, s_part, q0, cs.per, [&](int c, float s, float sq) {
+            const BnChanIn in = c == c_own ? pre[0] : bn_chan_in(p, c);
+            const int o = c - 4 * q0;
+            float mean, invstd;
+            bn_channel_stats(p, c, in, s, sq, mean, invstd);
+            bn_affine(in.gm, in.bt, mean, invstd, s_own[o], s_own[4 * cs.per + o]);
+        });
+        if (blockIdx.x == 0 && threadIdx.x == 0 && p.nbt != nullptr) *p.nbt = nbt0 + 1;
+        cluster_sync();
+        bn_cluster_gather(g, s_own, cs.per, s_ab);
+        cluster_arrive();
+    } else {
+        const bool last = bn_arrive(p.sync);
+        if (last) {
+            float* s_tot = s_ab;
+            bn_combine_partials(p.partial, g.nblk, g.C, s_tot, s_red);
+            float mean, invstd;
+#pragma unroll
+            for (int k = 0; k < kBnPre; ++k) {
+                const int c = threadIdx.x + k * kBnThreads;
+                if (c < g.C) bn_channel_stats(p, c, pre[k], s_tot[c], s_tot[g.C + c], mean, invstd);
+            }
+            for (int c = threadIdx.x + kBnPre * kBnThreads; c < g.C; c += kBnThreads)
+                bn_channel_stats(p, c, bn_chan_in(p, c), s_tot[c], s_tot[g.C + c], mean, invstd);
+            if (threadIdx.x == 0 && p.nbt != nullptr) *p.nbt = nbt0 + 1;
+        }
+        bn_release(p.sync, last, gen);
+        for (int c = threadIdx.x; c < g.C; c += kBnThreads)
+            bn_affine(__ldg(p.gamma + c), __ldg(p.beta + c), __ldcg(p.save_mean + c), __ldcg(p.save_invstd + c), s_ab[c],
+                      s_ab[g.C + c]);
     }
     __syncthreads();
 
@@ -266,6 +402,7 @@
             }
         }
     }
+    if (kCluster) cluster_wait();
 }
 
 struct BnBwdArgs {
@@ -281,11 +418,18 @@
     BnGeom g;
 };
 
-template <bool kPool>
+__device__ __forceinline__ float bn_per_row(float v, int M) { return (float)(v / (double)M); }
+__device__ __forceinline__ float4 bn_per_row(const float4& v, int M) {
+    return make_float4(bn_per_row(v.x, M), bn_per_row(v.y, M), bn_per_row(v.z, M), bn_per_row(v.w, M));
+}
+
+template <bool kPool, bool kCluster>
 __global__ void __launch_bounds__(kBnThreads) bn_bwd_kernel(const BnBwdArgs p) {
     extern __shared__ float4 s_dyn[];
     __shared__ float4 s_red[2 * kBnThreads];
     const BnGeom& g = p.g;
+    const BnClusterSmem cs = bn_cluster_smem(g, 2 * g.C, gridDim.x);
+    float* s_part = reinterpret_cast<float*>(s_dyn) + cs.part;
     const int tx = threadIdx.x % g.tpr, ty = threadIdx.x / g.tpr;
     const float4* x4 = reinterpret_cast<const float4*>(p.x);
     const float4* d4 = reinterpret_cast<const float4*>(p.dy);
@@ -307,9 +451,10 @@
         k.istd = __ldg(reinterpret_cast<const float4*>(p.save_invstd) + col);
         const float4 gm = __ldg(reinterpret_cast<const float4*>(p.gamma) + col);
         const float4 bt = __ldg(reinterpret_cast<const float4*>(p.beta) + col);
-        k.a = make_float4(__fmul_rn(gm.x, k.istd.x), __fmul_rn(gm.y, k.istd.y), __fmul_rn(gm.z, k.istd.z), __fmul_rn(gm.w, k.istd.w));
-        k.b = make_float4(__fsub_rn(bt.x, __fmul_rn(k.mean.x, k.a.x)), __fsub_rn(bt.y, __fmul_rn(k.mean.y, k.a.y)),
-                          __fsub_rn(bt.z, __fmul_rn(k.mean.z, k.a.z)), __fsub_rn(bt.w, __fmul_rn(k.mean.w, k.a.w)));
+        bn_affine(gm.x, bt.x, k.mean.x, k.istd.x, k.a.x, k.b.x);
+        bn_affine(gm.y, bt.y, k.mean.y, k.istd.y, k.a.y, k.b.y);
+        bn_affine(gm.z, bt.z, k.mean.z, k.istd.z, k.a.z, k.b.z);
+        bn_affine(gm.w, bt.w, k.mean.w, k.istd.w, k.a.w, k.b.w);
         return k;
     };
     auto mask = [&](const Col& k, const float4& v, float4& d) {
@@ -325,6 +470,7 @@
                            (v.w - k.mean.w) * k.istd.w);
     };
     float4 hx[kBnHold], hd[kBnHold];
+    const unsigned int gen = kCluster ? 0u : bn_gen(p.sync);
 
     for (int t = blockIdx.x; t < g.nblk; t += gridDim.x) {
         const bool held = g.hold && t == (int)blockIdx.x;
@@ -362,18 +508,34 @@
                     for (; r < row1; r += g.rpi) acc(__ldg(x4 + (size_t)r * g.cv + col), grad(row0, r, col));
                 }
             }
-            bn_tile_partial(sb, sg, tx, ty, col, g, s_red, p.partial, t);
-        }
-    }
-
-    unsigned int gen;
-    const bool last = bn_arrive(p.sync, gen);
-    if (last) {
-        float* s_tot = reinterpret_cast<float*>(s_dyn);
-        bn_combine_partials(p.partial, g.nblk, g.C, s_tot, s_red);
-        for (int c = threadIdx.x; c < g.C; c += kBnThreads) { p.dbeta[c] = s_tot[c]; p.dgamma[c] = s_tot[g.C + c]; }
-    }
-    bn_release(p.sync, last, gen);
+            if (kCluster) bn_tile_partial(sb, sg, tx, ty, col, g, s_red, s_part, t / gridDim.x);
+            else bn_tile_partial(sb, sg, tx, ty, col, g, s_red, p.partial, t);
+        }
+    }
+
+    if (kCluster) {
+        float* s_own = reinterpret_cast<float*>(s_dyn) + cs.own;
+        const int q0 = blockIdx.x * cs.per;
+        cluster_sync();
+        bn_cluster_combine(g, s_part, q0, cs.per, [&](int c, float db, float dg) {
+            p.dbeta[c] = db;
+            p.dgamma[c] = dg;
+            s_own[c - 4 * q0] = bn_per_row(db, g.M);
+            s_own[4 * cs.per + c - 4 * q0] = bn_per_row(dg, g.M);
+        });
+        cluster_sync();
+        bn_cluster_gather(g, s_own, cs.per, reinterpret_cast<float*>(s_dyn));
+        cluster_arrive();
+        __syncthreads();
+    } else {
+        const bool last = bn_arrive(p.sync);
+        if (last) {
+            float* s_tot = reinterpret_cast<float*>(s_dyn);
+            bn_combine_partials(p.partial, g.nblk, g.C, s_tot, s_red);
+            for (int c = threadIdx.x; c < g.C; c += kBnThreads) { p.dbeta[c] = s_tot[c]; p.dgamma[c] = s_tot[g.C + c]; }
+        }
+        bn_release(p.sync, last, gen);
+    }
 
     for (int t = blockIdx.x; t < g.nblk; t += gridDim.x) {
         const bool held = g.hold && t == (int)blockIdx.x;
@@ -382,11 +544,9 @@
             const int col = c0 + tx;
             if (ty >= g.rpi || col >= g.cv) continue;
             const Col k = column(col);
-            const float4 db = __ldcg(reinterpret_cast<const float4*>(p.dbeta) + col);
-            const float4 dg = __ldcg(reinterpret_cast<const float4*>(p.dgamma) + col);
-            const double M = (double)g.M;
-            const float4 mb = make_float4((float)(db.x / M), (float)(db.y / M), (float)(db.z / M), (float)(db.w / M));
-            const float4 mg = make_float4((float)(dg.x / M), (float)(dg.y / M), (float)(dg.z / M), (float)(dg.w / M));
+            const float4 mb = kCluster ? s_dyn[col] : bn_per_row(__ldcg(reinterpret_cast<const float4*>(p.dbeta) + col), g.M);
+            const float4 mg = kCluster ? s_dyn[g.cv + col]
+                                       : bn_per_row(__ldcg(reinterpret_cast<const float4*>(p.dgamma) + col), g.M);
             float4* o4 = reinterpret_cast<float4*>(p.dx);
             auto out = [&](size_t off, const float4& v, float4 d) {
                 const float4 xh = xhat(k, v);
@@ -411,6 +571,7 @@
             for (; r < row1; r += g.rpi) out((size_t)r * g.cv + col, __ldg(x4 + (size_t)r * g.cv + col), grad(row0, r, col));
         }
     }
+    if (kCluster) cluster_wait();
 }
 
 int bn_tile_rows(int M, int C) { return bn_geom(M, C).rows_per_block; }
@@ -428,21 +589,71 @@
     return base[dev] + 2 * (size_t)(slot % kBnSyncSlots);
 }
 
+constexpr int kBnClusterMax = 16;
+
 template <typename Args>
-static cudaError_t bn_launch(void (*kernel)(const Args), Args p, size_t smem, int max_ctas, cudaStream_t stream) {
+static bool bn_cluster_fits(void (*kernel)(const Args), int ctas, size_t smem) {
+    static std::mutex mu;
+    static std::map<std::tuple<const void*, int, int, size_t>, bool> known;
+    int dev = 0;
+    cudaGetDevice(&dev);
+    const auto key = std::make_tuple((const void*)kernel, dev, ctas, smem);
+    std::lock_guard<std::mutex> lock(mu);
+    const auto it = known.find(key);
+    if (it != known.end()) return it->second;
+    cudaError_t e = cudaSuccess;
+    if (ctas > 8) e = cudaFuncSetAttribute(kernel, cudaFuncAttributeNonPortableClusterSizeAllowed, 1);
+    if (e == cudaSuccess && smem > 32 * 1024)
+        e = cudaFuncSetAttribute(kernel, cudaFuncAttributeMaxDynamicSharedMemorySize, (int)smem);
+    int clusters = 0;
+    if (e == cudaSuccess) {
+        cudaLaunchConfig_t cfg = {};
+        cudaLaunchAttribute at[1];
+        at[0].id = cudaLaunchAttributeClusterDimension;
+        at[0].val.clusterDim.x = ctas; at[0].val.clusterDim.y = 1; at[0].val.clusterDim.z = 1;
+        cfg.gridDim = dim3(ctas); cfg.blockDim = dim3(kBnThreads); cfg.dynamicSmemBytes = smem;
+        cfg.attrs = at; cfg.numAttrs = 1;
+        e = cudaOccupancyMaxActiveClusters(&clusters, kernel, &cfg);
+    }
+    (void)cudaGetLastError();
+    return known[key] = e == cudaSuccess && clusters >= 1;
+}
+
+template <typename Args>
+static cudaError_t bn_launch(void (*grid_kernel)(const Args), void (*cluster_kernel)(const Args), Args p, size_t smem,
+                             int max_ctas, int cluster_tiles, BnLaunch* launched, cudaStream_t stream) {
+    const int cs = p.g.nblk < kBnClusterMax ? p.g.nblk : kBnClusterMax;
+    const size_t cluster_smem = sizeof(float) * bn_cluster_smem(p.g, (int)(smem / sizeof(float)), cs).end;
+    if (max_ctas <= 0 && p.g.nblk <= cluster_tiles && bn_cluster_fits(cluster_kernel, cs, cluster_smem)) {
+        if (cluster_smem > 32 * 1024) {
+            const cudaError_t e = cudaFuncSetAttribute(cluster_kernel, cudaFuncAttributeMaxDynamicSharedMemorySize, (int)cluster_smem);
+            if (e != cudaSuccess) return e;
+        }
+        cudaLaunchConfig_t cfg = {};
+        cudaLaunchAttribute at[1];
+        at[0].id = cudaLaunchAttributeClusterDimension;
+        at[0].val.clusterDim.x = cs; at[0].val.clusterDim.y = 1; at[0].val.clusterDim.z = 1;
+        cfg.gridDim = dim3(cs); cfg.blockDim = dim3(kBnThreads); cfg.dynamicSmemBytes = cluster_smem; cfg.stream = stream;
+        cfg.attrs = at; cfg.numAttrs = 1;
+        const cudaError_t e = cudaLaunchKernelEx(&cfg, cluster_kernel, p);
+        (void)cudaGetLastError();
+        if (launched != nullptr) *launched = BnLaunch{cs, cs};
+        return e;
+    }
     int dev = 0, sms = 0, per = 0;
     cudaGetDevice(&dev);
     cudaError_t e = cudaDeviceGetAttribute(&sms, cudaDevAttrMultiProcessorCount, dev);
     if (e == cudaSuccess && smem > 32 * 1024)
-        e = cudaFuncSetAttribute(kernel, cudaFuncAttributeMaxDynamicSharedMemorySize, (int)smem);
-    if (e == cudaSuccess) e = cudaOccupancyMaxActiveBlocksPerMultiprocessor(&per, kernel, kBnThreads, smem);
+        e = cudaFuncSetAttribute(grid_kernel, cudaFuncAttributeMaxDynamicSharedMemorySize, (int)smem);
+    if (e == cudaSuccess) e = cudaOccupancyMaxActiveBlocksPerMultiprocessor(&per, grid_kernel, kBnThreads, smem);
     if (e != cudaSuccess) return e;
     if (per < 1) return cudaErrorInvalidConfiguration;
     int grid = p.g.nblk < per * sms ? p.g.nblk : per * sms;
     if (max_ctas > 0 && grid > max_ctas) grid = max_ctas;
     void* args[] = {(void*)&p};
-    e = cudaLaunchCooperativeKernel((void*)kernel, dim3(grid), dim3(kBnThreads), args, smem, stream);
+    e = cudaLaunchCooperativeKernel((void*)grid_kernel, dim3(grid), dim3(kBnThreads), args, smem, stream);
     (void)cudaGetLastError();
+    if (launched != nullptr) *launched = BnLaunch{grid, 0};
     return e;
 }
 
@@ -457,24 +668,28 @@
 cudaError_t launch_bn_forward(const float* x, float* y, unsigned char* arg, float* partial, const float* gamma, const float* beta,
                               const float* cbias, float* save_mean, float* save_invstd, float* rmean, float* rvar, long long* nbt,
                               float momentum, float eps, int relu, int M, int C, int W, int slot, int max_ctas,
-                              cudaStream_t stream) {
+                              int cluster_tiles, BnLaunch* launched, cudaStream_t stream) {
     BnFwdArgs p{x, y, arg, partial, gamma, beta, cbias, save_mean, save_invstd, rmean, rvar, nbt, momentum, eps, relu, nullptr, {}};
     cudaError_t e = bn_prepare(p.g, p.sync, M, C, W, slot);
     if (e != cudaSuccess) return e;
     size_t smem = sizeof(float) * 2 * C;
     if (W > 0 && p.g.hold) smem += sizeof(float4) * p.g.rows_per_block * p.g.cv;
-    return W > 0 ? bn_launch(bn_fwd_kernel<true>, p, smem, max_ctas, stream) : bn_launch(bn_fwd_kernel<false>, p, smem, max_ctas, stream);
+    return W > 0 ? bn_launch(bn_fwd_kernel<true, false>, bn_fwd_kernel<true, true>, p, smem, max_ctas, cluster_tiles, launched, stream)
+                 : bn_launch(bn_fwd_kernel<false, false>, bn_fwd_kernel<false, true>, p, smem, max_ctas, cluster_tiles, launched,
+                             stream);
 }
 
 cudaError_t launch_bn_backward(const float* x, const float* dy, const unsigned char* arg, float* dx, float* partial,
                                const float* gamma, const float* beta, const float* save_mean, const float* save_invstd,
                                float* dgamma, float* dbeta, int relu, int M, int C, int W, int slot, int max_ctas,
-                               cudaStream_t stream) {
+                               int cluster_tiles, BnLaunch* launched, cudaStream_t stream) {
     BnBwdArgs p{x, dy, arg, dx, partial, gamma, beta, save_mean, save_invstd, dgamma, dbeta, relu, nullptr, {}};
     cudaError_t e = bn_prepare(p.g, p.sync, M, C, W, slot);
     if (e != cudaSuccess) return e;
     const size_t smem = sizeof(float) * 2 * C;
-    return W > 0 ? bn_launch(bn_bwd_kernel<true>, p, smem, max_ctas, stream) : bn_launch(bn_bwd_kernel<false>, p, smem, max_ctas, stream);
+    return W > 0 ? bn_launch(bn_bwd_kernel<true, false>, bn_bwd_kernel<true, true>, p, smem, max_ctas, cluster_tiles, launched, stream)
+                 : bn_launch(bn_bwd_kernel<false, false>, bn_bwd_kernel<false, true>, p, smem, max_ctas, cluster_tiles, launched,
+                             stream);
 }
 
 }
diff --git a/oktopk_b200/csrc/oktopk.cuh b/oktopk_b200/csrc/oktopk.cuh
--- a/oktopk_b200/csrc/oktopk.cuh
+++ b/oktopk_b200/csrc/oktopk.cuh
@@ -248,15 +248,16 @@
     int count;
 };
 cudaError_t launch_land(const LandParams& lp, float* bucket, cudaStream_t stream);
+struct BnLaunch { int ctas, cluster; };
 int bn_tile_rows(int M, int C);
 cudaError_t launch_bn_forward(const float* x, float* y, unsigned char* arg, float* partial, const float* gamma, const float* beta,
                               const float* cbias, float* save_mean, float* save_invstd, float* rmean, float* rvar, long long* nbt,
                               float momentum, float eps, int relu, int M, int C, int W, int slot, int max_ctas,
-                              cudaStream_t stream);
+                              int cluster_tiles, BnLaunch* launched, cudaStream_t stream);
 cudaError_t launch_bn_backward(const float* x, const float* dy, const unsigned char* arg, float* dx, float* partial,
                                const float* gamma, const float* beta, const float* save_mean, const float* save_invstd,
                                float* dgamma, float* dbeta, int relu, int M, int C, int W, int slot, int max_ctas,
-                               cudaStream_t stream);
+                               int cluster_tiles, BnLaunch* launched, cudaStream_t stream);
 cudaError_t launch_maxpool2_fwd(const float* x, float* y, unsigned char* arg, int N, int H, int W, int C, cudaStream_t stream);
 cudaError_t launch_maxpool2_bwd(const float* dy, const unsigned char* arg, float* dx, int N, int H, int W, int C,
                                 cudaStream_t stream);
diff --git a/oktopk_b200/ops/ext.py b/oktopk_b200/ops/ext.py
--- a/oktopk_b200/ops/ext.py
+++ b/oktopk_b200/ops/ext.py
@@ -29,7 +29,10 @@
                 n = max(1, (len(a[0]) + 95) // 96)
             LAUNCH_COUNT["total"] += n
             LAUNCH_COUNT[name] = LAUNCH_COUNT.get(name, 0) + n
-            return fn(*a, **kw)
+            r = fn(*a, **kw)
+            if name in ("bn_forward", "bn_backward") and r[1] > 0:
+                LAUNCH_COUNT[name + "_cluster"] = LAUNCH_COUNT.get(name + "_cluster", 0) + 1
+            return r
         return call
 
     def __getattr__(self, name):
diff --git a/oktopk_b200/ops/fused_bn.py b/oktopk_b200/ops/fused_bn.py
--- a/oktopk_b200/ops/fused_bn.py
+++ b/oktopk_b200/ops/fused_bn.py
@@ -9,6 +9,8 @@
 from . import ext
 
 MAX_CTAS = 0
+
+_CLUSTER_MAX_TILES = 4
 
 _SLOTS = itertools.count()
 
@@ -61,7 +63,7 @@
                      beta.data_ptr(), 0 if cbias is None else cbias.data_ptr(), stats.data_ptr(), stats.data_ptr() + 4 * Ch,
                      0 if rmean is None else rmean.data_ptr(), 0 if rvar is None else rvar.data_ptr(),
                      0 if nbt is None else nbt.data_ptr(), float(momentum), float(eps), int(relu), M, Ch,
-                     W if pool else 0, slot, MAX_CTAS, s)
+                     W if pool else 0, slot, MAX_CTAS, _CLUSTER_MAX_TILES, s)
         ctx.save_for_backward(x, gamma, beta, stats, arg)
         ctx.relu, ctx.pool, ctx.slot = bool(relu), bool(pool), slot
         return y
@@ -81,7 +83,8 @@
         s = torch.cuda.current_stream().cuda_stream
         C.bn_backward(x.data_ptr(), dy.data_ptr(), 0 if arg is None else arg.data_ptr(), dx.data_ptr(), partial.data_ptr(),
                       gamma.data_ptr(), beta.data_ptr(), stats.data_ptr(), stats.data_ptr() + 4 * Ch, dgb.data_ptr(),
-                      dgb.data_ptr() + 4 * Ch, int(ctx.relu), M, Ch, W if ctx.pool else 0, ctx.slot, MAX_CTAS, s)
+                      dgb.data_ptr() + 4 * Ch, int(ctx.relu), M, Ch, W if ctx.pool else 0, ctx.slot, MAX_CTAS,
+                      _CLUSTER_MAX_TILES, s)
         return dx, dgb[:Ch], dgb[Ch:], None, None, None, None, None, None, None, None, None
 
 
```
